# DmitryUlyanov/deep-image-prior

Measured on NVIDIA H100. Metric: optimisation iterations/sec (512x512 skip-net denoising, sum over independent images), higher is better.
Workload: dtype fp32 storage; tf32 tensor-core multiplies with fp32 accumulate in the convs (cuDNN's default fp32 mode)

## Files before the change

deep-image-prior_b200/csrc/conv_tc.cu:

```cuda
#include "conv_tc.cuh"
#include "ptx.cuh"
#include "wgmma.cuh"
#include "kernels.cuh"

namespace dip {

static constexpr int kTileM = 128;
static constexpr int kABytes = kTileM * 128;
static constexpr int kChunkBytes = kTileM * 128;
static constexpr int kNumThreads = 256;
static constexpr int kAccStride = kAccS;

struct SmemCtl {
  uint64_t full[8];
  uint64_t empty[8];
  float bias[160];
};

__host__ __device__ constexpr int round32(int n) { return (n + 31) & ~31; }
__host__ __device__ constexpr int round1024(int n) { return (n + 1023) & ~1023; }

template <bool BF16, int NT>
__device__ __forceinline__ void tc_conv_consumer(const TcConvParams& p, const TcConvParams* pm, SmemCtl* ctl,
                                                 uint8_t* stage_base, int stage_bytes, uint8_t* staging, int n_iters,
                                                 int tile0, int tile_stride, int num_tiles, int tiles_pp, int n_off) {
  const int et = threadIdx.x - 128;
  const int w = et >> 5, lane = et & 31;
  float acc[2][NT / 2];
  int stage = 0;
  uint32_t phase = 0;
  double stat_s1 = 0.0, stat_s2 = 0.0;
  const int bw_shift = 31 - __clz(p.bw);
  const uint32_t base_lo = desc_lo(smem_u32(stage_base));
  const uint32_t stage_step = static_cast<uint32_t>(stage_bytes) >> 4;
  constexpr uint32_t kBOff = static_cast<uint32_t>(kABytes) >> 4;
  constexpr uint32_t kHalfOff = (64u * 128u) >> 4;
  for (int it = 0; it < n_iters; ++it) {
    const int tile = tile0 + it * tile_stride;
    int tx = tile % p.tiles_x, ty = tile / p.tiles_x;
    int opx = 0, opy = 0;
    int kb_per_tile = p.kh * p.kw * p.kblocks;
    if (p.nphase > 0) {
      if (tile >= num_tiles) break;
      const int t = tile % tiles_pp;
      tx = t % p.tiles_x; ty = t / p.tiles_x;
      const TcConvParams::Phase& q = p.phs[tile / tiles_pp];
      opx = q.opx; opy = q.opy;
      kb_per_tile = q.kh * q.kw * p.kblocks;
    }
    const int x0 = tx * p.bw, y0 = ty * p.bh;
#pragma unroll
    for (int i = 0; i < NT / 2; ++i) { acc[0][i] = 0.f; acc[1][i] = 0.f; }
    int prev = -1;
    for (int kbt = 0; kbt < kb_per_tile; ++kbt) {
      mbar_wait(&ctl->full[stage], phase);
      const uint32_t a_lo = base_lo + stage * stage_step;
      const uint32_t b_lo = a_lo + kBOff;
      wgmma_fence();
#pragma unroll
      for (int k = 0; k < 4; ++k) {
        wgmma_ss<NT, BF16>(acc[0], desc_of(a_lo + 2 * k), desc_of(b_lo + 2 * k));
        wgmma_ss<NT, BF16>(acc[1], desc_of(a_lo + kHalfOff + 2 * k), desc_of(b_lo + 2 * k));
      }
      wgmma_commit();
      if (prev >= 0) {
        wgmma_wait<1>();
        if (lane == 0) mbar_arrive(&ctl->empty[prev]);
      }
      prev = stage;
      if (++stage == p.stages) { stage = 0; phase ^= 1; }
    }
    wgmma_wait<0>();
    if (prev >= 0 && lane == 0) mbar_arrive(&ctl->empty[prev]);

    if (et == 0) tma_store_wait_read0();
    named_bar_sync(1, 128);
#pragma unroll
    for (int h = 0; h < 2; ++h) {
#pragma unroll
      for (int j = 0; j < NT / 8; ++j) {
        const int col = 8 * j + 2 * (lane & 3);
        const int chunk = col >> 5;
        if (chunk < p.n_chunks) {
          const int q = (col & 31) >> 2, e = col & 3;
#pragma unroll
          for (int rr = 0; rr < 2; ++rr) {
            const int row = 64 * h + 16 * w + (lane >> 2) + 8 * rr;
            float2 o;
            o.x = acc[h][4 * j + 2 * rr] + ctl->bias[col];
            o.y = acc[h][4 * j + 2 * rr + 1] + ctl->bias[col + 1];
            *reinterpret_cast<float2*>(staging + chunk * kChunkBytes + row * 128 + ((q ^ (row & 7)) << 4) + e * 4) = o;
          }
        }
      }
    }
    fence_proxy_async_smem();
    named_bar_sync(1, 128);
    if (et == 0) {
      if (p.nphase > 0)
        for (int j = 0; j < p.n_chunks; ++j) tma_store_5d(&pm->tmD, staging + j * kChunkBytes, n_off + j * 32, opx, x0, opy, y0);
      else
        for (int j = 0; j < p.n_chunks; ++j) tma_store_3d(&pm->tmD, staging + j * kChunkBytes, n_off + j * 32, x0, y0);
      tma_store_commit();
    }
    if (p.stats != nullptr && et < p.n_mma) {
      const int c = et;
      const int j = c >> 5, q = (c & 31) >> 2, e = c & 3;
      const uint8_t* cb = staging + j * kChunkBytes + e * 4;
      float a0 = 0.f, a1 = 0.f, b0 = 0.f, b1 = 0.f;
      if (x0 + p.bw <= p.out_w && y0 + p.bh <= p.out_h) {
#pragma unroll 8
        for (int m = 0; m < kTileM; m += 2) {
          const float x = *reinterpret_cast<const float*>(cb + m * 128 + ((q ^ (m & 7)) << 4));
          const float y = *reinterpret_cast<const float*>(cb + (m + 1) * 128 + ((q ^ ((m + 1) & 7)) << 4));
          a0 += x; b0 = fmaf(x, x, b0);
          a1 += y; b1 = fmaf(y, y, b1);
        }
      } else {
        for (int m = 0; m < kTileM; ++m) {
          const int py = m >> bw_shift, px = m & (p.bw - 1);
          if (x0 + px < p.out_w && y0 + py < p.out_h) {
            const float x = *reinterpret_cast<const float*>(cb + m * 128 + ((q ^ (m & 7)) << 4));
            a0 += x; b0 = fmaf(x, x, b0);
          }
        }
      }
      stat_s1 += static_cast<double>(a0 + a1);
      stat_s2 += static_cast<double>(b0 + b1);
    }
  }
  if (p.stats != nullptr && et < p.n_mma && n_off + et < p.stats_ld) {
    const int rep = (blockIdx.x % kAccR) * kAccLine;
    atomicAdd(&p.stats[(n_off + et) * kAccStride + rep], stat_s1);
    atomicAdd(&p.stats[(p.stats_ld + n_off + et) * kAccStride + rep], stat_s2);
  }
  if (et == 0) tma_store_wait_all0();
}

template <bool DEEP, bool BF16 = false>
__device__ __forceinline__ void tc_conv_body(const TcConvParams& p, const TcConvParams* pm, uint8_t* smem_raw) {
  constexpr int KE = BF16 ? 64 : 32;
  const int grid_x = DEEP ? p.vgrid : static_cast<int>(gridDim.x);
  if (DEEP && static_cast<int>(blockIdx.x) >= grid_x) return;
  uint8_t* smem = reinterpret_cast<uint8_t*>((reinterpret_cast<uintptr_t>(smem_raw) + 1023) & ~uintptr_t(1023));
  const int nt = round32(p.n_mma);
  const int b_bytes = p.n_mma * 128;
  const int stage_bytes = kABytes + round1024(nt * 128);
  uint8_t* stage_base = smem;
  uint8_t* staging = stage_base + p.stages * stage_bytes;
  SmemCtl* ctl = reinterpret_cast<SmemCtl*>(staging + p.n_chunks * kChunkBytes);

  const int warp = threadIdx.x >> 5;
  const int lane = threadIdx.x & 31;
  const int tiles_pp = p.tiles_x * p.tiles_y;
  const int num_tiles = p.nphase > 0 ? tiles_pp * p.nphase : tiles_pp;
  const int n_split = p.n_split < 1 ? 1 : p.n_split;
  const int n_part = blockIdx.x % n_split;
  const int n_off = n_part * p.n_mma;
  const int n_total = p.n_mma * n_split;
  const int tile_stride = grid_x / n_split;
  const int n_iters = (num_tiles + tile_stride - 1) / tile_stride;
  const int tile0 = blockIdx.x / n_split;

  if (!DEEP) pdl_trigger();
  if (warp == 0 && lane == 0) {
    tma_prefetch_desc(&pm->tmA);
    tma_prefetch_desc(&pm->tmB);
    tma_prefetch_desc(&pm->tmD);
  }
  if (warp == 1 && lane == 0) {
    for (int i = 0; i < p.stages; ++i) {
      mbar_init(&ctl->full[i], 1);
      mbar_init(&ctl->empty[i], 4);
    }
    fence_mbar_init();
  }
  if (!DEEP) pdl_wait();
  if (warp == 3) {
    for (int i = lane; i < 160; i += 32)
      ctl->bias[i] = (p.bias != nullptr && i < p.n_mma && (p.n_valid == 0 || n_off + i < p.n_valid)) ? p.bias[n_off + i] : 0.f;
  }
  __syncthreads();

  if (warp == 0) {
    int stage = 0;
    uint32_t phase = 0;
    for (int it = 0; it < n_iters; ++it) {
      const int tile = tile0 + it * tile_stride;
      int kh = p.kh, kw = p.kw, offx = p.offx, offy = p.offy, tap0 = 0;
      int x0 = (tile % p.tiles_x) * p.bw, y0 = (tile / p.tiles_x) * p.bh;
      if (p.nphase > 0) {
        if (tile >= num_tiles) break;
        const TcConvParams::Phase& q = p.phs[tile / tiles_pp];
        const int t = tile % tiles_pp;
        kh = q.kh; kw = q.kw; offx = q.offx; offy = q.offy; tap0 = q.tap0;
        x0 = (t % p.tiles_x) * p.bw; y0 = (t / p.tiles_x) * p.bh;
      }
      for (int r = 0; r < kh; ++r) {
        for (int s = 0; s < kw; ++s) {
          const int ix = offx + s, iy = offy + r;
          int cpx, cx, cpy, cy;
          if (p.stride == 1) {
            cpx = 0; cx = x0 + ix; cpy = 0; cy = y0 + iy;
          } else {
            cpx = ix & 1; cx = x0 + (ix >> 1); cpy = iy & 1; cy = y0 + (iy >> 1);
          }
          const int tap = tap0 + r * kw + s;
          for (int kb = 0; kb < p.kblocks; ++kb) {
            mbar_wait(&ctl->empty[stage], phase ^ 1);
            uint8_t* sa = stage_base + stage * stage_bytes;
            if (elect_one()) {
              mbar_expect_tx(&ctl->full[stage], kABytes + b_bytes);
              tma_load_5d(sa, &pm->tmA, &ctl->full[stage], kb * KE, cpx, cx, cpy, cy);
              tma_load_2d(sa + kABytes, &pm->tmB, &ctl->full[stage], kb * KE, tap * n_total + n_off);
            }
            __syncwarp();
            if (++stage == p.stages) { stage = 0; phase ^= 1; }
          }
        }
      }
    }
  } else if (warp >= 4) {
    switch (nt) {
      case 32: tc_conv_consumer<BF16, 32>(p, pm, ctl, stage_base, stage_bytes, staging, n_iters, tile0, tile_stride, num_tiles, tiles_pp, n_off); break;
      case 64: tc_conv_consumer<BF16, 64>(p, pm, ctl, stage_base, stage_bytes, staging, n_iters, tile0, tile_stride, num_tiles, tiles_pp, n_off); break;
      case 96: tc_conv_consumer<BF16, 96>(p, pm, ctl, stage_base, stage_bytes, staging, n_iters, tile0, tile_stride, num_tiles, tiles_pp, n_off); break;
      case 128: tc_conv_consumer<BF16, 128>(p, pm, ctl, stage_base, stage_bytes, staging, n_iters, tile0, tile_stride, num_tiles, tiles_pp, n_off); break;
      default: tc_conv_consumer<BF16, 160>(p, pm, ctl, stage_base, stage_bytes, staging, n_iters, tile0, tile_stride, num_tiles, tiles_pp, n_off); break;
    }
  }
  __syncthreads();
}
__global__ void __launch_bounds__(kNumThreads, 1) tc_conv_kernel(const __grid_constant__ TcConvParams p) {
  extern __shared__ __align__(1024) uint8_t smem_raw[];
  tc_conv_body<false>(p, &p, smem_raw);
}
__global__ void __launch_bounds__(kNumThreads, 1) tc_conv_kernel_bf16(const __grid_constant__ TcConvParams p) {
  extern __shared__ __align__(1024) uint8_t smem_raw[];
  tc_conv_body<false, true>(p, &p, smem_raw);
}

struct SmemCtlW {
  uint64_t full[8];
  uint64_t empty[8];
  uint64_t bt_full[2];
  uint64_t bt_empty[2];
};

__host__ __device__ constexpr int wgrad_tbuf_bytes(bool bf16, int n_cols) {
  return (bf16 ? kTileM * 128 : 0) + round1024(n_cols * 128);
}


template <int NT>
__device__ __forceinline__ void tc_wgrad_transposer(const TcWgradParams& p, SmemCtlW* ctl, uint32_t stage_base, int stage_bytes,
                                                    uint32_t bt_base, int items) {
  constexpr int kBt = wgrad_tbuf_bytes(false, NT);
  constexpr int kUnitsO = ((NT + 31) / 32) * 8;
  constexpr int kIters = (kUnitsO + 11) / 12;
  constexpr int y_bytes = 4 * kWgradKp * 128;
  const int tt = threadIdx.x - 32;
  const int lane = threadIdx.x & 31;
  const int b = tt & 7, b0 = b & 1, b1 = (b >> 1) & 1, b2 = b >> 2;
  uint32_t src[kIters], dst[kIters], sq[kIters], dq[kIters];
  bool ok[kIters];
#pragma unroll
  for (int it = 0; it < kIters; ++it) {
    const int o = (tt >> 3) + 12 * it;
    const int kk = (b1 ^ (o & 1)) | ((b2 ^ ((o >> 1) & 1)) << 1);
    const int c4 = (o >> 3) * 8 + b2 * 4 + b1 * 2 + ((o >> 2) & 1);
    ok[it] = o < kUnitsO && c4 < NT / 4;
    src[it] = y_bytes + (c4 >> 3) * (kWgradKp * 128) + (8 * kk + b0) * 128;
    sq[it] = (c4 & 7) ^ b0;
    dst[it] = c4 * 4 * 128;
    dq[it] = (2 * kk + b0) ^ ((c4 & 1) << 2);
  }
  int stage = 0, tb = 0;
  uint32_t phase = 0, tphase = 0;
  for (int item = blockIdx.x; item < items; item += gridDim.x) {
    const int ks = item % p.ksplits;
    const int blk0 = static_cast<int>((static_cast<long long>(p.px_blocks) * ks) / p.ksplits);
    const int blk1 = static_cast<int>((static_cast<long long>(p.px_blocks) * (ks + 1)) / p.ksplits);
    for (int blk = blk0; blk < blk1; ++blk) {
      mbar_wait(&ctl->full[stage], phase);
      mbar_wait(&ctl->bt_empty[tb], tphase ^ 1);
      const uint32_t sx = stage_base + stage * stage_bytes;
      const uint32_t bt = bt_base + tb * kBt;
#pragma unroll
      for (int it = 0; it < kIters; ++it) {
        if (ok[it]) {
          uint4 v[4];
#pragma unroll
          for (int i = 0; i < 4; ++i) v[i] = lds128(sx + src[it] + 256 * i + ((sq[it] ^ (2 * i)) << 4));
          sts128(bt + dst[it] + ((dq[it] ^ 0) << 4), v[0].x, v[1].x, v[2].x, v[3].x);
          sts128(bt + dst[it] + 128 + ((dq[it] ^ 1) << 4), v[0].y, v[1].y, v[2].y, v[3].y);
          sts128(bt + dst[it] + 256 + ((dq[it] ^ 2) << 4), v[0].z, v[1].z, v[2].z, v[3].z);
          sts128(bt + dst[it] + 384 + ((dq[it] ^ 3) << 4), v[0].w, v[1].w, v[2].w, v[3].w);
        }
      }
      fence_proxy_async_smem();
      mbar_arrive(&ctl->bt_full[tb]);
      __syncwarp();
      if (lane == 0) mbar_arrive(&ctl->empty[stage]);
      if (++stage == p.stages) { stage = 0; phase ^= 1; }
      tb ^= 1;
      if (tb == 0) tphase ^= 1;
    }
  }
}

template <int NT, bool DOUBLE>
__device__ __forceinline__ void tc_wgrad_mma(const TcWgradParams& p, SmemCtlW* ctl, uint32_t stage_base, int stage_bytes,
                                             uint32_t bt_base, int items) {
  constexpr int kBt = wgrad_tbuf_bytes(false, NT);
  constexpr bool kDouble = DOUBLE && NT <= 136;
  const int et = threadIdx.x - 128;
  const int w = et >> 5, lane = et & 31, g = lane >> 2, t = lane & 3;
  const int taps = p.kh * p.kw;
  uint32_t aoff[4];
#pragma unroll
  for (int r = 0; r < 4; ++r) {
    const int hi = r & 1, e = r >> 1;
    const int q = 4 * (w & 1) + (g >> 2) + 2 * hi, px = 2 * t + e;
    aoff[r] = (w >> 1) * (kWgradKp * 128) + px * 128 + ((q ^ px) << 4) + (g & 3) * 4;
  }
  auto load_a = [&](uint32_t (&f)[8][4], uint32_t sy) {
#pragma unroll
    for (int h = 0; h < 2; ++h)
#pragma unroll
      for (int kk = 0; kk < 4; ++kk)
#pragma unroll
        for (int r = 0; r < 4; ++r) f[4 * h + kk][r] = lds32(sy + aoff[r] + h * 2 * (kWgradKp * 128) + kk * 1024);
  };
  int stage = 0, tb = 0;
  uint32_t phase = 0, tphase = 0;
  bool pending = false;
  float acc[2][NT / 2];
  uint32_t fa[8][4], fb[8][4];
  auto step = [&](uint32_t (&cur)[8][4], uint32_t (&nxt)[8][4], bool more) {
    mbar_wait(&ctl->bt_full[tb], tphase);
    const uint32_t b_lo = desc_lo(bt_base + tb * kBt);
    wgmma_fence();
#pragma unroll
    for (int kk = 0; kk < 4; ++kk) {
      wgmma_rs<NT>(acc[0], cur[kk], desc_of(b_lo + 2 * kk));
      wgmma_rs<NT>(acc[1], cur[4 + kk], desc_of(b_lo + 2 * kk));
    }
    wgmma_commit();
    __syncwarp();
    if (lane == 0) mbar_arrive(&ctl->empty[stage]);
    if (++stage == p.stages) { stage = 0; phase ^= 1; }
    if constexpr (kDouble) wgmma_wait<1>(); else wgmma_wait<0>();
    if (pending && lane == 0) mbar_arrive(&ctl->bt_empty[tb ^ 1]);
    pending = true;
    tb ^= 1;
    if (tb == 0) tphase ^= 1;
    if (more) {
      mbar_wait(&ctl->full[stage], phase);
      load_a(nxt, stage_base + stage * stage_bytes);
    }
  };
  for (int item = blockIdx.x; item < items; item += gridDim.x) {
    const int tap = item / p.ksplits, ks = item % p.ksplits;
    const int blk0 = static_cast<int>((static_cast<long long>(p.px_blocks) * ks) / p.ksplits);
    const int blk1 = static_cast<int>((static_cast<long long>(p.px_blocks) * (ks + 1)) / p.ksplits);
#pragma unroll
    for (int i = 0; i < NT / 2; ++i) { acc[0][i] = 0.f; acc[1][i] = 0.f; }
    if (blk0 < blk1) {
      mbar_wait(&ctl->full[stage], phase);
      load_a(fa, stage_base + stage * stage_bytes);
    }
    for (int blk = blk0; blk < blk1; blk += 2) {
      step(fa, kDouble ? fb : fa, blk + 1 < blk1);
      if (blk + 1 == blk1) break;
      step(kDouble ? fb : fa, fa, blk + 2 < blk1);
    }
    wgmma_wait<0>();
    if (pending && lane == 0) mbar_arrive(&ctl->bt_empty[tb ^ 1]);
    pending = false;
    float* dst = p.partial + (static_cast<size_t>(ks) * taps + tap) * 128 * NT;
#pragma unroll
    for (int h = 0; h < 2; ++h) {
#pragma unroll
      for (int j = 0; j < NT / 8; ++j) {
        const int col = 8 * j + 2 * t;
#pragma unroll
        for (int rr = 0; rr < 2; ++rr) {
          const int n = 64 * h + 16 * w + g + 8 * rr;
          *reinterpret_cast<float2*>(dst + static_cast<size_t>(n) * NT + col) =
              make_float2(acc[h][4 * j + 2 * rr], acc[h][4 * j + 2 * rr + 1]);
        }
      }
    }
  }
}

template <int NT>
__device__ __forceinline__ void tc_wgrad_consumer_bf16(const TcWgradParams& p, SmemCtlW* ctl, uint8_t* smem, int stage_bytes,
                                                       uint8_t* tbase, int items) {
  constexpr int KE = 64;
  constexpr int E = 2;
  constexpr int kTA = kTileM * 128;
  constexpr int kTBuf = wgrad_tbuf_bytes(true, NT);
  constexpr int kRows = 128 + NT;
  const int et = threadIdx.x - 128;
  const int w = et >> 5, lane = et & 31;
  constexpr int chunk_bytes = kWgradKp * 128;
  constexpr int y_bytes = (128 / KE) * chunk_bytes;
  constexpr int groups = kWgradKp * E / 16;
  constexpr int nk = kWgradKp / 16;
  const int taps = p.kh * p.kw;
  int stage = 0, tb = 0;
  uint32_t phase = 0;
  float acc[2][NT / 2];
  for (int item = blockIdx.x; item < items; item += gridDim.x) {
    const int tap = item / p.ksplits, ks = item % p.ksplits;
    const int blk0 = static_cast<int>((static_cast<long long>(p.px_blocks) * ks) / p.ksplits);
    const int blk1 = static_cast<int>((static_cast<long long>(p.px_blocks) * (ks + 1)) / p.ksplits);
#pragma unroll
    for (int i = 0; i < NT / 2; ++i) { acc[0][i] = 0.f; acc[1][i] = 0.f; }
    for (int blk = blk0; blk < blk1; ++blk) {
      mbar_wait(&ctl->full[stage], phase);
      named_bar_sync(1, 128);
      const uint8_t* sy = smem + stage * stage_bytes;
      const uint8_t* sx = sy + y_bytes;
      uint8_t* ta = tbase + tb * kTBuf;
      uint8_t* tbb = ta + kTA;
      for (int i = et; i < kRows * groups; i += 128) {
        const int g = i / kRows, row = i % kRows;
        const bool is_y = row < 128;
        const int rs = is_y ? row : row - 128;
        const uint8_t* src = (is_y ? sy : sx) + (rs / KE) * chunk_bytes;
        const int cb = (rs % KE) * E;
        uint32_t v[4];
#pragma unroll
        for (int u = 0; u < 4; ++u) {
          const int px = g * 8 + 2 * u;
          const uint32_t lo = *reinterpret_cast<const uint16_t*>(src + px * 128 + ((((cb >> 4) ^ (px & 7)) << 4) | (cb & 15)));
          const uint32_t hi = *reinterpret_cast<const uint16_t*>(src + (px + 1) * 128 + ((((cb >> 4) ^ ((px + 1) & 7)) << 4) | (cb & 15)));
          v[u] = lo | (hi << 16);
        }
        uint8_t* dst = (is_y ? ta : tbb) + rs * 128 + ((g ^ (rs & 7)) << 4);
        *reinterpret_cast<uint4*>(dst) = make_uint4(v[0], v[1], v[2], v[3]);
      }
      fence_proxy_async_smem();
      named_bar_sync(1, 128);
      if (lane == 0) mbar_arrive(&ctl->empty[stage]);
      const uint32_t a_lo = desc_lo(smem_u32(ta)), b_lo = desc_lo(smem_u32(tbb));
      wgmma_fence();
#pragma unroll
      for (int k = 0; k < nk; ++k) {
        wgmma_ss<NT, true>(acc[0], desc_of(a_lo + 2 * k), desc_of(b_lo + 2 * k));
        wgmma_ss<NT, true>(acc[1], desc_of(a_lo + ((64u * 128u) >> 4) + 2 * k), desc_of(b_lo + 2 * k));
      }
      wgmma_commit();
      wgmma_wait<1>();
      tb ^= 1;
      if (++stage == p.stages) { stage = 0; phase ^= 1; }
    }
    wgmma_wait<0>();
    float* dst = p.partial + (static_cast<size_t>(ks) * taps + tap) * 128 * NT;
#pragma unroll
    for (int h = 0; h < 2; ++h) {
#pragma unroll
      for (int j = 0; j < NT / 8; ++j) {
        const int col = 8 * j + 2 * (lane & 3);
#pragma unroll
        for (int rr = 0; rr < 2; ++rr) {
          const int n = 64 * h + 16 * w + (lane >> 2) + 8 * rr;
          *reinterpret_cast<float2*>(dst + static_cast<size_t>(n) * NT + col) =
              make_float2(acc[h][4 * j + 2 * rr], acc[h][4 * j + 2 * rr + 1]);
        }
      }
    }
  }
}

template <bool DEEP, bool BF16, int NT>
__device__ __forceinline__ void tc_wgrad_role(const TcWgradParams& p, SmemCtlW* ctl, uint8_t* smem, int stage_bytes,
                                              uint8_t* tbase, int items, int warp) {
  if constexpr (BF16) {
    if (warp >= 4) tc_wgrad_consumer_bf16<NT>(p, ctl, smem, stage_bytes, tbase, items);
  } else {
    if (warp >= 4) tc_wgrad_mma<NT, !DEEP>(p, ctl, smem_u32(smem), stage_bytes, smem_u32(tbase), items);
    else tc_wgrad_transposer<NT>(p, ctl, smem_u32(smem), stage_bytes, smem_u32(tbase), items);
  }
}

template <bool DEEP, bool BF16 = false>
__device__ __forceinline__ void tc_wgrad_body(const TcWgradParams& p, const TcWgradParams* pm, uint8_t* smem_raw) {
  uint8_t* smem = reinterpret_cast<uint8_t*>((reinterpret_cast<uintptr_t>(smem_raw) + 1023) & ~uintptr_t(1023));
  constexpr int KE = BF16 ? 64 : 32;
  constexpr int YCH = 128 / KE;
  constexpr int chunk_bytes = kWgradKp * 128;
  const int y_bytes = YCH * chunk_bytes;
  const int x_bytes = p.c_chunks * chunk_bytes;
  const int stage_bytes = y_bytes + x_bytes;
  uint8_t* tbase = smem + p.stages * stage_bytes;
  SmemCtlW* ctl = reinterpret_cast<SmemCtlW*>(tbase + 2 * wgrad_tbuf_bytes(BF16, p.n_cols));
  const int items = p.kh * p.kw * p.ksplits;

  const int warp = threadIdx.x >> 5;
  const int lane = threadIdx.x & 31;
  if (!DEEP) pdl_trigger();
  if (warp == 0 && lane == 0) {
    tma_prefetch_desc(&pm->tmY);
    tma_prefetch_desc(&pm->tmX);
  }
  if (warp == 1 && lane == 0) {
    for (int i = 0; i < p.stages; ++i) {
      mbar_init(&ctl->full[i], 1);
      mbar_init(&ctl->empty[i], BF16 ? 4 : 7);
    }
    for (int i = 0; i < 2; ++i) {
      mbar_init(&ctl->bt_full[i], 96);
      mbar_init(&ctl->bt_empty[i], 4);
    }
    fence_mbar_init();
  }
  if (!DEEP) pdl_wait();
  __syncthreads();

  if (warp == 0) {
    int stage = 0;
    uint32_t phase = 0;
    for (int item = blockIdx.x; item < items; item += gridDim.x) {
      const int tap = item / p.ksplits, ks = item % p.ksplits;
      const int r = tap / p.kw, s = tap % p.kw;
      const int blk0 = static_cast<int>((static_cast<long long>(p.px_blocks) * ks) / p.ksplits);
      const int blk1 = static_cast<int>((static_cast<long long>(p.px_blocks) * (ks + 1)) / p.ksplits);
      const int ix = p.offx + s, iy = p.offy + r;
      for (int blk = blk0; blk < blk1; ++blk) {
        const int y = blk / p.px_blocks_x;
        const int x0 = (blk % p.px_blocks_x) * kWgradKp;
        int cpx, cx, cpy, cy;
        if (p.stride == 1) {
          cpx = 0; cx = x0 + ix; cpy = 0; cy = y + iy;
        } else {
          cpx = ix & 1; cx = x0 + (ix >> 1); cpy = iy & 1; cy = y + (iy >> 1);
        }
        mbar_wait(&ctl->empty[stage], phase ^ 1);
        uint8_t* sy = smem + stage * stage_bytes;
        if (elect_one()) {
          mbar_expect_tx(&ctl->full[stage], stage_bytes);
          for (int j = 0; j < YCH; ++j) tma_load_3d(sy + j * chunk_bytes, &pm->tmY, &ctl->full[stage], j * KE, x0, y);
          for (int j = 0; j < p.c_chunks; ++j)
            tma_load_5d(sy + y_bytes + j * chunk_bytes, &pm->tmX, &ctl->full[stage], j * KE, cpx, cx, cpy, cy);
        }
        __syncwarp();
        if (++stage == p.stages) { stage = 0; phase ^= 1; }
      }
    }
  } else {
    switch (p.n_cols) {
      case 32: tc_wgrad_role<DEEP, BF16, 32>(p, ctl, smem, stage_bytes, tbase, items, warp); break;
      case 64: tc_wgrad_role<DEEP, BF16, 64>(p, ctl, smem, stage_bytes, tbase, items, warp); break;
      case 96: tc_wgrad_role<DEEP, BF16, 96>(p, ctl, smem, stage_bytes, tbase, items, warp); break;
      case 128: tc_wgrad_role<DEEP, BF16, 128>(p, ctl, smem, stage_bytes, tbase, items, warp); break;
      case 136: tc_wgrad_role<DEEP, BF16, 136>(p, ctl, smem, stage_bytes, tbase, items, warp); break;
      default: tc_wgrad_role<DEEP, BF16, 160>(p, ctl, smem, stage_bytes, tbase, items, warp); break;
    }
  }
  __syncthreads();
}
__global__ void __launch_bounds__(kNumThreads, 1) tc_wgrad_kernel(const __grid_constant__ TcWgradParams p) {
  extern __shared__ __align__(1024) uint8_t smem_raw[];
  tc_wgrad_body<false>(p, &p, smem_raw);
}
__global__ void __launch_bounds__(kNumThreads, 1) tc_wgrad_kernel_bf16(const __grid_constant__ TcWgradParams p) {
  extern __shared__ __align__(1024) uint8_t smem_raw[];
  tc_wgrad_body<false, true>(p, &p, smem_raw);
}

static constexpr size_t kMaxSmem = 232448;

size_t tc_conv_smem_bytes(const TcConvParams& p) {
  const size_t b_bytes = round1024(round32(p.n_mma) * 128);
  return 1024 + p.stages * (kABytes + b_bytes) + static_cast<size_t>(p.n_chunks) * kChunkBytes + sizeof(SmemCtl);
}
size_t tc_wgrad_smem_bytes(const TcWgradParams& p) {
  const size_t chunk = static_cast<size_t>(kWgradKp) * 128;
  const size_t tbuf = wgrad_tbuf_bytes(p.bf16 != 0, p.n_cols);
  return 1024 + p.stages * ((p.bf16 ? 2 : 4) * chunk + static_cast<size_t>(p.c_chunks) * chunk) + 2 * tbuf + sizeof(SmemCtlW);
}

cudaError_t tc_kernels_init() {
  cudaError_t e = cudaFuncSetAttribute(tc_conv_kernel, cudaFuncAttributeMaxDynamicSharedMemorySize, (int)kMaxSmem);
  if (e != cudaSuccess) return e;
  e = cudaFuncSetAttribute(tc_conv_kernel_bf16, cudaFuncAttributeMaxDynamicSharedMemorySize, (int)kMaxSmem);
  if (e != cudaSuccess) return e;
  e = cudaFuncSetAttribute(tc_wgrad_kernel_bf16, cudaFuncAttributeMaxDynamicSharedMemorySize, (int)kMaxSmem);
  if (e != cudaSuccess) return e;
  return cudaFuncSetAttribute(tc_wgrad_kernel, cudaFuncAttributeMaxDynamicSharedMemorySize, (int)kMaxSmem);
}

static bool conv_params_ok(const TcConvParams& p) {
  return p.n_mma >= 1 && p.n_mma <= 160 && p.n_chunks == (p.n_mma + 31) / 32 && p.stages >= 1 && p.stages <= 8 &&
         p.kblocks >= 1 && p.nphase >= 0 && p.nphase <= 4 &&
         (p.bw & (p.bw - 1)) == 0 && p.bw * p.bh == kTileM;
}

cudaError_t tc_conv_launch(const TcConvParams& p, int num_sms, cudaStream_t s) {
  if (!conv_params_ok(p)) return cudaErrorInvalidValue;
  const int tiles = p.tiles_x * p.tiles_y * (p.nphase > 0 ? p.nphase : 1);
  int grid = tiles < num_sms ? tiles : num_sms;
  if (p.n_split > 1) {
    if (tiles * p.n_split > num_sms) return cudaErrorInvalidValue;
    grid = tiles * p.n_split;
  }
  const size_t smem = tc_conv_smem_bytes(p);
  if (smem > kMaxSmem) return cudaErrorInvalidValue;
  return launch_k(p.bf16 ? tc_conv_kernel_bf16 : tc_conv_kernel, dim3(grid), dim3(kNumThreads), smem, s, 1, p);
}
int tc_conv_grid(const TcConvParams& p, int num_sms) {
  const int tiles = p.tiles_x * p.tiles_y * (p.nphase > 0 ? p.nphase : 1);
  if (p.n_split > 1) return tiles * p.n_split;
  return tiles < num_sms ? tiles : num_sms;
}

cudaError_t tc_wgrad_launch(const TcWgradParams& p, cudaStream_t s) {
  const size_t smem = tc_wgrad_smem_bytes(p);
  const bool cols_ok = p.n_cols == 32 || p.n_cols == 64 || p.n_cols == 96 || p.n_cols == 128 || p.n_cols == 136 ||
                       p.n_cols == 160;
  if (smem > kMaxSmem || !cols_ok || p.n_cols > p.c_chunks * (p.bf16 ? 64 : 32) || p.stages < 1 || p.stages > 8)
    return cudaErrorInvalidValue;
  return launch_k(p.bf16 ? tc_wgrad_kernel_bf16 : tc_wgrad_kernel, dim3(p.kh * p.kw * p.ksplits), dim3(kNumThreads), smem, s, 1, p);
}

}
```

deep-image-prior_b200/csrc/conv_tc.cuh:

```cuda
#pragma once
#include <cuda.h>
#include <cuda_runtime.h>
#include <stdint.h>

namespace dip {

struct TcConvParams {
  CUtensorMap tmA;
  CUtensorMap tmB;
  CUtensorMap tmD;
  int tiles_x, tiles_y;
  int bw, bh;
  int out_w, out_h;
  int kh, kw;
  int stride;
  int offx, offy;
  int bf16;
  int kblocks;
  int n_mma;
  int n_chunks;
  int stages;
  int n_split;
  int vgrid;
  int nphase;
  struct Phase { int kh, kw, offx, offy, tap0, opx, opy; } phs[4];
  int n_valid;
  const float* bias;
  double* stats;
  int stats_ld;
};

static constexpr int kWgradKp = 32;
struct TcWgradParams {
  CUtensorMap tmY;
  CUtensorMap tmX;
  float* partial;
  int kh, kw, stride, offx, offy;
  int px_blocks_x;
  int px_blocks;
  int bf16;
  int c_chunks;
  int n_cols;
  int ksplits;
  int stages;
};

size_t tc_conv_smem_bytes(const TcConvParams& p);
size_t tc_wgrad_smem_bytes(const TcWgradParams& p);
cudaError_t tc_conv_launch(const TcConvParams& p, int num_sms, cudaStream_t s);
cudaError_t tc_wgrad_launch(const TcWgradParams& p, cudaStream_t s);
int tc_conv_grid(const TcConvParams& p, int num_sms);
cudaError_t tc_kernels_init();

}
```

deep-image-prior_b200/csrc/engine.cu:

```cuda
#include <cuda.h>
#include <cuda_bf16.h>
#include <cuda_runtime.h>
#include <math.h>
#include <stdio.h>
#include <stdlib.h>
#include <string.h>

#include <initializer_list>
#include <map>
#include <string>
#include <vector>

#include "../../include/dip.h"
#include "conv_tc.cuh"
#include "deep.cuh"
#include "kernels.cuh"

namespace dip {

static thread_local std::string g_err;
static int fail(const std::string& m) {
  g_err = m;
  return -1;
}
#define DIP_CUDA(expr)                                                                                   \
  do {                                                                                                   \
    cudaError_t _e = (expr);                                                                             \
    if (_e != cudaSuccess) return fail(std::string(#expr) + ": " + cudaGetErrorString(_e));              \
  } while (0)
#define DIP_CHECK(expr)        \
  do {                         \
    int _r = (expr);           \
    if (_r != 0) return _r;    \
  } while (0)

typedef CUresult (*PFN_encodeTiled)(CUtensorMap*, CUtensorMapDataType, cuuint32_t, void*, const cuuint64_t*,
                                    const cuuint64_t*, const cuuint32_t*, const cuuint32_t*, CUtensorMapInterleave,
                                    CUtensorMapSwizzle, CUtensorMapL2promotion, CUtensorMapFloatOOBfill);
static PFN_encodeTiled g_encode = nullptr;
static int g_num_sms = 0;
static unsigned long long g_inited_mask = 0;

static int engine_init() {
  int dev = 0;
  DIP_CUDA(cudaGetDevice(&dev));
  if (dev >= 64) return fail("dip: device ordinal >= 64 not supported");
  if (g_inited_mask & (1ull << dev)) return 0;
  cudaDeviceProp prop;
  DIP_CUDA(cudaGetDeviceProperties(&prop, dev));
  if (prop.major != 9 || prop.minor != 0)
    return fail("dip requires an sm_90 (H100) device; found sm_" + std::to_string(prop.major * 10 + prop.minor));
  g_num_sms = prop.multiProcessorCount;
  void* fn = nullptr;
  cudaDriverEntryPointQueryResult q;
  DIP_CUDA(cudaGetDriverEntryPoint("cuTensorMapEncodeTiled", &fn, cudaEnableDefault, &q));
  if (fn == nullptr || q != cudaDriverEntryPointSuccess) return fail("cuTensorMapEncodeTiled not available from the driver");
  g_encode = reinterpret_cast<PFN_encodeTiled>(fn);
  DIP_CUDA(tc_kernels_init());
  DIP_CUDA(down_kernels_init());
  DIP_CUDA(deep_kernels_init());
  g_inited_mask |= 1ull << dev;
  return 0;
}

static bool is_tc(int prec) { return prec == DIP_PRECISION_TF32 || prec == DIP_PRECISION_BF16; }

static int encode_map(CUtensorMap* m, const void* base, int rank, const cuuint64_t* dims, const cuuint64_t* strides_b,
                      const cuuint32_t* box, bool bf16 = false) {
  cuuint32_t estr[5] = {1, 1, 1, 1, 1};
  CUresult r = g_encode(m, bf16 ? CU_TENSOR_MAP_DATA_TYPE_BFLOAT16 : CU_TENSOR_MAP_DATA_TYPE_FLOAT32, rank, const_cast<void*>(base), dims, strides_b, box, estr,
                        CU_TENSOR_MAP_INTERLEAVE_NONE, CU_TENSOR_MAP_SWIZZLE_128B,
                        CU_TENSOR_MAP_L2_PROMOTION_L2_128B,
                        CU_TENSOR_MAP_FLOAT_OOB_FILL_NONE);
  if (r != CUDA_SUCCESS) {
    char buf[256];
    snprintf(buf, sizeof buf, "cuTensorMapEncodeTiled failed (%d): rank %d dims %llu %llu %llu box %u %u %u", (int)r, rank,
             (unsigned long long)dims[0], (unsigned long long)dims[1], (unsigned long long)(rank > 2 ? dims[2] : 0), box[0],
             box[1], rank > 2 ? box[2] : 0);
    return fail(buf);
  }
  return 0;
}
static int map_act5(CUtensorMap* m, const void* base, int rows, int cols, int ld, int c, int stride, int bw, int bh,
                    bool bf16 = false) {
  const cuuint64_t e = bf16 ? 2 : sizeof(float);
  cuuint64_t dims[5], str[4];
  if (stride == 1) {
    dims[0] = c; dims[1] = 1; dims[2] = cols; dims[3] = 1; dims[4] = rows;
    str[0] = ld * e; str[1] = ld * e; str[2] = (cuuint64_t)cols * ld * e; str[3] = (cuuint64_t)cols * ld * e;
  } else {
    dims[0] = c; dims[1] = 2; dims[2] = cols / 2; dims[3] = 2; dims[4] = rows / 2;
    str[0] = ld * e; str[1] = 2 * ld * e; str[2] = (cuuint64_t)cols * ld * e; str[3] = 2 * (cuuint64_t)cols * ld * e;
  }
  cuuint32_t box[5] = {bf16 ? 64u : 32u, 1, (cuuint32_t)bw, 1, (cuuint32_t)bh};
  return encode_map(m, base, 5, dims, str, box, bf16);
}
static int map_act3(CUtensorMap* m, const void* base, int rows, int cols, int ld, int c, int bw, int bh, bool bf16 = false) {
  const cuuint64_t e = bf16 ? 2 : sizeof(float);
  cuuint64_t dims[3] = {(cuuint64_t)c, (cuuint64_t)cols, (cuuint64_t)rows};
  cuuint64_t str[2] = {ld * e, (cuuint64_t)cols * ld * e};
  cuuint32_t box[3] = {bf16 ? 64u : 32u, (cuuint32_t)bw, (cuuint32_t)bh};
  return encode_map(m, base, 3, dims, str, box, bf16);
}
static int map_w2(CUtensorMap* m, const void* base, int rows_total, int kcols, int box_rows, bool bf16 = false) {
  const cuuint64_t e = bf16 ? 2 : sizeof(float);
  cuuint64_t dims[2] = {(cuuint64_t)kcols, (cuuint64_t)rows_total};
  cuuint64_t str[1] = {kcols * e};
  cuuint32_t box[2] = {bf16 ? 64u : 32u, (cuuint32_t)box_rows};
  return encode_map(m, base, 2, dims, str, box, bf16);
}

static void pick_tile(int w, int h, int* bw, int* bh) {
  const int cand[5][2] = {{128, 1}, {64, 2}, {32, 4}, {16, 8}, {8, 16}};
  long long best = -1;
  for (int i = 0; i < 5; ++i) {
    const long long cw = (w + cand[i][0] - 1) / cand[i][0] * cand[i][0];
    const long long ch = (h + cand[i][1] - 1) / cand[i][1] * cand[i][1];
    const long long cost = cw * ch * 64 + (cand[i][0] + cand[i][1]);
    if (best < 0 || cost < best) { best = cost; *bw = cand[i][0]; *bh = cand[i][1]; }
  }
}
static int round_up(int x, int m) { return (x + m - 1) / m * m; }
struct Timer {
  bool on = false;
  std::vector<cudaEvent_t> pool;
  size_t used = 0;
  struct Rec { int cls; double flops; size_t e0, e1; };
  std::vector<Rec> recs;
  size_t get(cudaStream_t s) {
    if (used == pool.size()) { cudaEvent_t e; cudaEventCreate(&e); pool.push_back(e); }
    cudaEventRecord(pool[used], s);
    return used++;
  }
  void reset() { used = 0; recs.clear(); }
};
struct TimeScope {
  Timer* t; int cls; double flops; size_t e0 = 0; cudaStream_t s;
  TimeScope(Timer* t_, int cls_, double flops_, cudaStream_t s_) : t(t_ && t_->on ? t_ : nullptr), cls(cls_), flops(flops_), s(s_) {
    if (t) e0 = t->get(s);
  }
  ~TimeScope() { if (t) { size_t e1 = t->get(s); t->recs.push_back({cls, flops, e0, e1}); } }
};

enum HbmId { H_INPUT_PAD = 0, H_NOISE, H_SKINNY_FWD, H_BN_ACT_WRITE, H_BN_ACT_HEAD, H_CAT_STATS, H_CAT_WRITE, H_BN_BWD_REDUCE,
             H_BN_BWD_APPLY, H_CAT_BWD_REDUCE, H_CAT_BWD_APPLY, H_UPADJ, H_SKINNY_BWD, H_MSE, H_ADAM, H_HEAD_DLOGIT, H_DOWN_FWD,
             H_DOWN_BWD, H_PACK, H_WGRAD_REDUCE };
#define HBM_T(timer, id, sub, bytes, s, stmt)                                              \
  do {                                                                                     \
    TimeScope _ts((timer), 16 + 8 * (int)(id) + (int)(sub), (double)(bytes), (s));         \
    stmt;                                                                                  \
  } while (0)

static int pick_nsplit(int tiles, int n_rows) {
  int mx = 4;
  if (const char* e = getenv("DIP_NSPLIT_MAX")) mx = atoi(e);
  int sp = 1;
  while (sp * 2 <= mx && tiles * sp * 2 <= g_num_sms && n_rows % (32 * sp * 2) == 0) sp *= 2;
  return sp;
}
static void fit_stages(TcConvParams& p, size_t budget = 232448) {
  p.stages = 6;
  while (tc_conv_smem_bytes(p) > budget && p.stages > 2) p.stages--;
}
struct ConvOp {
  Timer* timer = nullptr;
  double alg_flops() const { return 2.0 * out_h * out_w * (double)N * C * k * k; }
  int N = 128, C = 0, k = 1, stride = 1, rot = 0;
  int Np = 128;
  int n_pad = 128;
  int n_pad16 = 128;
  int Ctot = 0, coff = 0;
  bool do_fprop = true, do_wgrad = true;
  int dg_ld = 0;
  int c_pad = 0;
  int crows = 0;
  bool bf16 = false;
  int c_pad16 = 0;
  const uint16_t* in16 = nullptr; int in_ld16 = 0;
  const uint16_t* dg_in16 = nullptr;
  const uint16_t* wg_dy16 = nullptr;
  const float* in = nullptr; int in_rows = 0, in_cols = 0, in_ld = 0; int offx = 0, offy = 0;
  float* out = nullptr; int out_h = 0, out_w = 0;
  double* stats = nullptr;
  float* wp_f = nullptr; float* wp_d = nullptr;
  float* wacc = nullptr;
  bool has_dgrad = false;
  bool dg_s2 = false;
  const float* dg_in = nullptr; int dg_in_h = 0, dg_in_w = 0;
  float* dg_out = nullptr; int dg_out_h = 0, dg_out_w = 0; int dg_off = 0;
  const float* wg_dy = nullptr; int wg_h = 0, wg_w = 0;
  int p_w = -1, p_b = -1;
  TcConvParams fp{}, dg{};
  TcWgradParams wg{};
  int simt_ksplits = 1;

  void set_shapes() {
    c_pad = round_up(C, 32);
    c_pad16 = round_up(C, 64);
    crows = round_up(C, 16);
    Np = round_up(N, 16); n_pad = round_up(N, 32); n_pad16 = round_up(N, 64);
    if (Ctot == 0) Ctot = C;
    if (dg_ld == 0) dg_ld = C;
  }
  size_t wp_f_elems() const { return (size_t)k * k * Np * c_pad; }
  size_t wp_d_elems() const { return (size_t)k * k * crows * n_pad; }
  size_t wacc_elems() const { return (size_t)tc_ksplits() * k * k * 128 * wg_cols(); }
  int wg_cols() const { return C > 128 && C <= 136 ? 136 : c_pad; }
  int tc_ksplits() const {
    const int blocks = wg_h * ((wg_w + kWgradKp - 1) / kWgradKp);
    int ks = static_cast<int>(kNumSms) / (k * k);
    if (ks > blocks) ks = blocks;
    return ks < 1 ? 1 : ks;
  }
  size_t partial_elems(int prec) const {
    return is_tc(prec) ? wacc_elems() : (size_t)simt_ksplits * k * k * 128 * c_pad;
  }

  int build_tc(float* partial) {
    int bw, bh;
    pick_tile(out_w, out_h, &bw, &bh);
    fp = TcConvParams{};
    if (do_fprop) {
    DIP_CHECK(bf16 ? map_act5(&fp.tmA, in16, in_rows, in_cols, in_ld16, C, stride, bw, bh, true)
                   : map_act5(&fp.tmA, in, in_rows, in_cols, in_ld, C, stride, bw, bh));
    fp.n_split = pick_nsplit(((out_w + bw - 1) / bw) * ((out_h + bh - 1) / bh), Np);
    DIP_CHECK(map_w2(&fp.tmB, wp_f, k * k * Np, bf16 ? c_pad16 : c_pad, Np / fp.n_split, bf16));
    DIP_CHECK(map_act3(&fp.tmD, out, out_h, out_w, N, N, bw, bh));
    fp.tiles_x = (out_w + bw - 1) / bw; fp.tiles_y = (out_h + bh - 1) / bh;
    fp.bw = bw; fp.bh = bh; fp.out_w = out_w; fp.out_h = out_h;
    fp.kh = fp.kw = k; fp.stride = stride; fp.offx = offx; fp.offy = offy;
    fp.bf16 = bf16 ? 1 : 0;
    fp.kblocks = bf16 ? c_pad16 / 64 : c_pad / 32;
    fp.n_mma = Np / fp.n_split; fp.n_chunks = (fp.n_mma + 31) / 32;
    fp.n_valid = N;
    fp.bias = nullptr; fp.stats = stats; fp.stats_ld = N;
    fit_stages(fp);
    }
    if (has_dgrad && dg_s2) {
      const int gh = dg_out_h / 2, gw = dg_out_w / 2;
      pick_tile(gw, gh, &bw, &bh);
      dg = TcConvParams{};
      DIP_CHECK(bf16 ? map_act5(&dg.tmA, dg_in16, dg_in_h, dg_in_w, N, N, 1, bw, bh, true)
                     : map_act5(&dg.tmA, dg_in, dg_in_h, dg_in_w, N, N, 1, bw, bh));
      dg.n_split = pick_nsplit(4 * ((gw + bw - 1) / bw) * ((gh + bh - 1) / bh), crows);
      DIP_CHECK(map_w2(&dg.tmB, wp_d, k * k * crows, bf16 ? n_pad16 : n_pad, crows / dg.n_split, bf16));
      DIP_CHECK(map_act5(&dg.tmD, dg_out, dg_out_h, dg_out_w, dg_ld, C, 2, bw, bh));
      dg.tiles_x = (gw + bw - 1) / bw; dg.tiles_y = (gh + bh - 1) / bh;
      dg.bw = bw; dg.bh = bh; dg.out_w = gw; dg.out_h = gh;
      dg.kh = dg.kw = 2; dg.stride = 1; dg.offx = dg.offy = -1;
      dg.nphase = 4;
      int t0 = 0;
      for (int a = 0; a < 2; ++a)
        for (int b = 0; b < 2; ++b) {
          TcConvParams::Phase& q = dg.phs[a * 2 + b];
          q.kh = 2 - a; q.kw = 2 - b; q.offy = a == 0 ? -1 : 0; q.offx = b == 0 ? -1 : 0; q.tap0 = t0; q.opx = b; q.opy = a;
          t0 += q.kh * q.kw;
        }
      dg.bf16 = bf16 ? 1 : 0;
      dg.kblocks = bf16 ? n_pad16 / 64 : n_pad / 32;
      dg.n_mma = crows / dg.n_split; dg.n_chunks = (dg.n_mma + 31) / 32;
      dg.bias = nullptr; dg.stats = nullptr; dg.stats_ld = 0;
      fit_stages(dg);
    } else if (has_dgrad) {
      pick_tile(dg_out_w, dg_out_h, &bw, &bh);
      dg = TcConvParams{};
      DIP_CHECK(bf16 ? map_act5(&dg.tmA, dg_in16, dg_in_h, dg_in_w, N, N, 1, bw, bh, true)
                     : map_act5(&dg.tmA, dg_in, dg_in_h, dg_in_w, N, N, 1, bw, bh));
      dg.n_split = pick_nsplit(((dg_out_w + bw - 1) / bw) * ((dg_out_h + bh - 1) / bh), crows);
      DIP_CHECK(map_w2(&dg.tmB, wp_d, k * k * crows, bf16 ? n_pad16 : n_pad, crows / dg.n_split, bf16));
      DIP_CHECK(map_act3(&dg.tmD, dg_out, dg_out_h, dg_out_w, dg_ld, C, bw, bh));
      dg.tiles_x = (dg_out_w + bw - 1) / bw; dg.tiles_y = (dg_out_h + bh - 1) / bh;
      dg.bw = bw; dg.bh = bh; dg.out_w = dg_out_w; dg.out_h = dg_out_h;
      dg.kh = dg.kw = k; dg.stride = 1; dg.offx = dg.offy = dg_off;
      dg.bf16 = bf16 ? 1 : 0;
      dg.kblocks = bf16 ? n_pad16 / 64 : n_pad / 32;
      dg.n_mma = crows / dg.n_split; dg.n_chunks = (dg.n_mma + 31) / 32;
      dg.bias = nullptr; dg.stats = nullptr; dg.stats_ld = 0;
      fit_stages(dg);
    }
    wg = TcWgradParams{};
    if (!do_wgrad) return 0;
    wg.bf16 = bf16 ? 1 : 0;
    if (bf16) {
      DIP_CHECK(map_act3(&wg.tmY, wg_dy16, wg_h, wg_w, N, N, kWgradKp, 1, true));
      DIP_CHECK(map_act5(&wg.tmX, in16, in_rows, in_cols, in_ld16, C, stride, kWgradKp, 1, true));
    } else {
      DIP_CHECK(map_act3(&wg.tmY, wg_dy, wg_h, wg_w, N, N, kWgradKp, 1));
      DIP_CHECK(map_act5(&wg.tmX, in, in_rows, in_cols, in_ld, C, stride, kWgradKp, 1));
    }
    wg.partial = partial;
    wg.kh = wg.kw = k; wg.stride = stride; wg.offx = offx; wg.offy = offy;
    wg.px_blocks_x = (wg_w + kWgradKp - 1) / kWgradKp;
    wg.px_blocks = wg_h * wg.px_blocks_x;
    wg.c_chunks = bf16 ? c_pad16 / 64 : c_pad / 32;
    wg.n_cols = wg_cols();
    wg.ksplits = tc_ksplits();
    wg.stages = 6;
    while (tc_wgrad_smem_bytes(wg) > 232448 && wg.stages > 1) wg.stages--;
    if (tc_wgrad_smem_bytes(wg) > 232448) return fail("wgrad stage does not fit in shared memory");
    return 0;
  }

  int run_fprop(int prec, const float* bias, cudaStream_t s) {
    if (is_tc(prec)) {
      TcConvParams p = fp;
      p.bias = bias;
      TimeScope ts(timer, 0, alg_flops(), s);
      DIP_CUDA(tc_conv_launch(p, g_num_sms, s));
    } else {
      SimtConvArgs a{};
      a.A = in; a.a_h = in_rows; a.a_w = in_cols; a.a_ld = in_ld; a.a_c = C;
      a.Wp = wp_f; a.n_rows = Np; a.c_pad = c_pad;
      a.D = out; a.d_h = out_h; a.d_w = out_w; a.d_ld = N; a.d_c = N;
      a.kh = a.kw = k; a.stride = stride; a.offx = offx; a.offy = offy; a.bias = bias;
      launch_simt_conv(a, s);
      if (stats != nullptr) launch_channel_stats(out, N, N, out_h * out_w, stats, s);
      DIP_CUDA(cudaGetLastError());
    }
    return 0;
  }
  int run_dgrad(int prec, cudaStream_t s) {
    if (is_tc(prec)) {
      TimeScope ts(timer, 1, alg_flops(), s);
      DIP_CUDA(tc_conv_launch(dg, g_num_sms, s));
    } else {
      SimtConvArgs a{};
      a.A = dg_in; a.a_h = dg_in_h; a.a_w = dg_in_w; a.a_ld = N; a.a_c = N;
      a.Wp = wp_d; a.n_rows = crows; a.c_pad = n_pad;
      a.D = dg_out; a.d_h = dg_out_h; a.d_w = dg_out_w; a.d_ld = dg_ld; a.d_c = C;
      a.kh = a.kw = k; a.stride = 1; a.offx = a.offy = dg_off; a.bias = nullptr;
      launch_simt_conv(a, s);
      DIP_CUDA(cudaGetLastError());
    }
    return 0;
  }
  int run_wgrad(int prec, float* partial, float* dw, cudaStream_t s) {
    static const bool dbg_skip = getenv("DIP_DBG_SKIP_WGRAD") != nullptr;
    if (dbg_skip) return 0;
    int ks;
    if (is_tc(prec)) {
      TcWgradParams p = wg;
      p.partial = wacc != nullptr ? wacc : partial;
      {
        TimeScope ts(timer, 2, alg_flops(), s);
        DIP_CUDA(tc_wgrad_launch(p, s));
      }
      if (wacc != nullptr) return 0;
      launch_wgrad_reduce(partial, p.ksplits, N, C, k, k, rot, p.n_cols, dw, s, Ctot, coff);
      DIP_CUDA(cudaGetLastError());
      return 0;
    } else {
      SimtWgradArgs a{};
      a.dY = wg_dy; a.h = wg_h; a.w = wg_w; a.dy_ld = N; a.n = N;
      a.X = in; a.x_h = in_rows; a.x_w = in_cols; a.x_ld = in_ld; a.x_c = C;
      a.kh = a.kw = k; a.stride = stride; a.offx = offx; a.offy = offy;
      a.partial = partial; a.c_pad = c_pad; a.ksplits = ks = simt_ksplits;
      launch_simt_wgrad(a, s);
    }
    HBM_T(timer, H_WGRAD_REDUCE, 0, ((double)ks + 1.0) * k * k * 128.0 * c_pad * sizeof(float), s,
          launch_wgrad_reduce(partial, ks, N, C, k, k, rot, c_pad, dw, s, Ctot, coff));
    DIP_CUDA(cudaGetLastError());
    return 0;
  }
};

struct PackEntry {
  const float* w; float* dst_f; float* dst_d;
  int N, C, k, rot, n_rows, c_pad, c_rows;
  int Ctot, coff;
  int s2;
  int bf16;
  int c_pad16;
  int n_pad;
};
__constant__ int kS2Taps[9] = {2 * 3 + 2, 2 * 3 + 0, 0 * 3 + 2, 0 * 3 + 0,
                               2 * 3 + 1, 0 * 3 + 1,
                               1 * 3 + 2, 1 * 3 + 0,
                               1 * 3 + 1};
__global__ void k_pack_table(const PackEntry* __restrict__ tab) {
  pdl_enter();
  const PackEntry e = tab[blockIdx.y];
  const int taps = e.k * e.k;
  const int c_pad = e.bf16 ? e.c_pad16 : e.c_pad;
  __nv_bfloat16* const f16 = reinterpret_cast<__nv_bfloat16*>(e.dst_f);
  __nv_bfloat16* const d16 = reinterpret_cast<__nv_bfloat16*>(e.dst_d);
  const long long nf = e.dst_f != nullptr ? (long long)taps * e.n_rows * c_pad : 0;
  const int n_pad = e.n_pad > 0 ? e.n_pad : 128;
  const long long nd = e.dst_d != nullptr ? (long long)taps * e.c_rows * n_pad : 0;
  for (long long i = (long long)blockIdx.x * blockDim.x + threadIdx.x; i < nf + nd; i += (long long)gridDim.x * blockDim.x) {
    if (i < nf) {
      const int c = (int)(i % c_pad), n = (int)((i / c_pad) % e.n_rows), tap = (int)(i / ((long long)c_pad * e.n_rows));
      float v = 0.f;
      if (n < e.N && c < e.C) v = e.w[((long long)n * e.Ctot + (c + e.coff + e.rot) % e.Ctot) * taps + tap];
      if (e.bf16) f16[i] = __float2bfloat16_rn(v); else e.dst_f[i] = v;
    } else {
      const long long j = i - nf;
      const int n = (int)(j % n_pad), c = (int)((j / n_pad) % e.c_rows), tapf = (int)(j / ((long long)n_pad * e.c_rows));
      const int tap = e.s2 ? kS2Taps[tapf] : taps - 1 - tapf;
      float v = 0.f;
      if (n < e.N && c < e.C) v = e.w[((long long)n * e.Ctot + (c + e.coff + e.rot) % e.Ctot) * taps + tap];
      if (e.bf16) d16[j] = __float2bfloat16_rn(v); else e.dst_d[j] = v;
    }
  }
}
struct UnpackEntry {
  const float* acc; float* dw;
  int N, C, taps, rot, cols, Ctot, coff, ks;
};
__global__ void k_wgrad_unpack_table(const UnpackEntry* __restrict__ tab) {
  pdl_enter();
  const UnpackEntry e = tab[blockIdx.y];
  const int total = e.N * e.C * e.taps;
  for (int i = blockIdx.x * blockDim.x + threadIdx.x; i < total; i += gridDim.x * blockDim.x) {
    const int tap = i % e.taps, c = (i / e.taps) % e.C, n = i / (e.taps * e.C);
    const size_t split = (size_t)e.taps * 128 * e.cols;
    const float* src = e.acc + ((size_t)tap * 128 + n) * e.cols + c;
    float v = 0.f;
    for (int k = 0; k < e.ks; ++k) v += src[k * split];
    e.dw[((size_t)n * e.Ctot + (c + e.coff + e.rot) % e.Ctot) * e.taps + tap] = v;
  }
}
struct CvtEntry {
  const double* src; float* dst; int n, rot;
  int row, row_ld;
};
__global__ void k_cvt_table(const CvtEntry* __restrict__ tab) {
  pdl_enter();
  const CvtEntry e = tab[blockIdx.x];
  for (int i = threadIdx.x; i < e.n; i += blockDim.x) {
    const int si = e.row > 0 ? (i / e.row) * e.row_ld + i % e.row : i;
    e.dst[(i + e.rot) % e.n] = (float)acc_get(e.src + (size_t)si * kAccS);
  }
}
struct RunEntry {
  const double* fwd; float* rm; float* rv; void* nb; int C, rot; float n; int nb_is_float;
};
__global__ void k_running_table(const RunEntry* __restrict__ tab) {
  pdl_enter();
  const RunEntry e = tab[blockIdx.x];
  if (e.rm == nullptr) return;
  for (int c = threadIdx.x; c < e.C; c += blockDim.x) {
    const int ct = (c + e.rot) % e.C;
    const double m = acc_get(e.fwd + c * kAccS) / e.n;
    double var = acc_get(e.fwd + (e.C + c) * kAccS) / e.n - m * m;
    if (var < 0) var = 0;
    const double unb = e.n > 1.f ? var * e.n / (e.n - 1.0) : var;
    e.rm[ct] = 0.9f * e.rm[ct] + 0.1f * (float)m;
    e.rv[ct] = 0.9f * e.rv[ct] + 0.1f * (float)unb;
  }
  if (threadIdx.x == 0 && e.nb != nullptr) {
    if (e.nb_is_float) *reinterpret_cast<float*>(e.nb) += 1.f; else *reinterpret_cast<long long*>(e.nb) += 1;
  }
}

struct Arena {
  uint8_t* base;
  size_t off = 0;
  template <typename T>
  T* get(size_t n) {
    off = (off + 255) & ~size_t(255);
    T* p = base ? reinterpret_cast<T*>(base + off) : nullptr;
    off += n * sizeof(T);
    return p;
  }
};
struct BufInfo {
  void* ptr; int rows, cols, ld, c;
};
struct BnLayer {
  int C = 0, rot = 0; float n = 1.f;
  double* fwd = nullptr; double* bwd = nullptr; double* dbias = nullptr;
  int p_gamma = -1, p_beta = -1, p_bias = -1, idx = -1;
};
struct Level {
  int H, W, h, w, Cin;
  int Cin_act;
  int bilinear;
  int nd = 128, nu = 128, ns = 0, cu = 128;
  float *rawF = nullptr, *dRawF = nullptr;
  uint16_t* dRawF16 = nullptr;
  float *Pin, *raw_s, *raw_d1, *P_d1, *raw_d2, *P_d2, *P_cat, *raw_u, *A_u, *raw_v, *U;
  uint16_t *Pin16 = nullptr, *P_d1_16 = nullptr, *P_d2_16 = nullptr, *P_cat16 = nullptr, *A_u16 = nullptr;
  uint16_t *dRaw_v16 = nullptr, *dRaw_u16 = nullptr, *dRaw_d2_16 = nullptr, *dRaw_d1_16 = nullptr, *dRaw_s16 = nullptr;
  int Pin_ld16 = 0, cat_ld16 = 0;
  float *dUp;
  float *dS;
  float *dRaw_v, *dA_u, *dRaw_u, *dP_cat, *dCat, *dRaw_s, *dRaw_d2, *dP_d1, *dRaw_d1, *ZS, *dPin;
  BnLayer bn_s, bn_d1, bn_d2, bn_cat, bn_u, bn_v;
  int p_skip_w, p_skip_b;
  double* dw_s;
  ConvOp d1, d2, up, c11;
  ConvOp sk, up_a, up_b;
};

}

using namespace dip;

struct dip_plan {
  dip_net_desc desc;
  int H, W;
  int zero_pad = 0;
  bool dry = false;
  uint8_t* ws = nullptr;
  size_t ws_bytes = 0;
  std::vector<Level> lv;
  std::vector<long long> numel;
  std::vector<float*> params, grads;
  std::vector<void*> running;
  std::vector<BnLayer*> bns;
  std::vector<ConvOp*> convs;
  std::map<std::string, BufInfo> bufs;
  int p_head_w = -1, p_head_b = -1;
  double* dw_head = nullptr; double* db_head = nullptr; double* db_scratch = nullptr;
  float* out_saved = nullptr;
  double* acc_fwd = nullptr; size_t acc_fwd_n = 0;
  double* acc_bwd = nullptr; size_t acc_bwd_n = 0;
  float* partial = nullptr;
  float* zbuf = nullptr; float* dout = nullptr; float* dl4 = nullptr;
  static constexpr int kDownMaxK = 64;
  float* ds_kern = nullptr;
  float* ds_y = nullptr;
  float* ds_dy = nullptr;
  int ds_K = 0, ds_f = 1, ds_pad = 0, ds_Ho = 0, ds_Wo = 0;
  static constexpr int kLossRing = 65536;
  double* loss_ring = nullptr;
  int* it_dev = nullptr;
  struct GraphKey {
    const void *z0 = nullptr, *target = nullptr, *mask = nullptr, *out = nullptr, *slots = nullptr;
    unsigned long long adam_id = 0, adam_bind = 0;
    float sigma = 0.f; uint64_t seed = 0; double lr = 0.0;
    bool operator==(const GraphKey& o) const {
      return z0 == o.z0 && target == o.target && mask == o.mask && out == o.out && slots == o.slots && adam_id == o.adam_id &&
             adam_bind == o.adam_bind && sigma == o.sigma && seed == o.seed && lr == o.lr;
    }
  };
  GraphKey gkey{};
  cudaGraphExec_t gexec = nullptr;
  cudaGraphExec_t gfwd = nullptr, gbwd = nullptr;
  cudaStream_t gstream = nullptr;
  cudaEvent_t gev_in = nullptr, gev_out = nullptr;
  cudaStream_t wstream = nullptr;
  cudaStream_t sstream = nullptr;
  std::vector<cudaEvent_t> wev;
  size_t wev_used = 0;
  bool side_on = false;
  std::vector<dip::ConvOp*> deferred;
  struct { bool on = false; const float* z0 = nullptr; float sigma = 0.f; uint64_t seed = 0, offset = 0; const int* it_dev = nullptr; } fnoise;
  bool prepacked = false;
  PackEntry* d_pack = nullptr; CvtEntry* d_cvt = nullptr; RunEntry* d_run = nullptr; UnpackEntry* d_unpack = nullptr;
  int n_pack = 0, n_cvt = 0, n_run = 0, n_unpack = 0;
  float* wacc_base = nullptr; size_t wacc_bytes = 0;
  static constexpr int kDeepMaxOps = 96;
  DeepOp* d_deep_fwd = nullptr; DeepOp* d_deep_bwd = nullptr;
  int n_deep_fwd = 0, n_deep_bwd = 0, deep_grid = 0, deep_from = 2;
  unsigned* deep_bar = nullptr;
  long long pack_max = 0;
  bool bound = false;
  int nbt_is_float = 0;
  int launches_fwd = 0, launches_bwd = 0;
  Timer timer;
};

namespace dip {

static BnRef bn_ref(const dip_plan* P, const BnLayer& b) {
  BnRef r;
  r.fwd = b.fwd; r.gamma = P->params[b.p_gamma]; r.beta = P->params[b.p_beta];
  r.C = b.C; r.rot = b.rot; r.inv_n = 1.f / b.n;
  return r;
}

static int build_plan(dip_plan* P, Arena& A) {
  const dip_net_desc& d = P->desc;
  const int L = d.num_scales;
  if (L < 1 || L > 8) return fail("dip-b200: 1..8 scales supported");
  std::vector<int> ND(L), NU(L), NS(L);
  for (int l = 0; l < L; ++l) {
    ND[l] = d.channels > 0 ? d.channels : d.channels_down[l];
    NU[l] = d.channels > 0 ? d.channels : d.channels_up[l];
    NS[l] = d.channels > 0 ? d.skip_channels : d.channels_skip[l];
    for (int w : {ND[l], NU[l]})
      if (w < 8 || w > 128 || w % 8 != 0)
        return fail("dip-b200: num_channels_down / num_channels_up must be multiples of 8 in [8, 128] (128 in the BASELINE configurations)");
  }
  bool wide = true, uniform = true;
  for (int l = 0; l < L; ++l) {
    wide = wide && NS[l] == 128 && ND[l] == 128 && NU[l] == 128;
    uniform = uniform && ND[l] == 128 && NU[l] == 128 && NS[l] == NS[0];
  }
  for (int l = 0; l < L; ++l)
    if (!(wide || NS[l] == 0 || NS[l] == 4))
      return fail("dip-b200: num_channels_skip must be 0 or 4 per scale, or 128 at every scale of a 128-wide network");
  const int CS = NS[0];
  if (d.downsample_mode != 0 && d.downsample_mode != 1) return fail("dip-b200: downsample_mode must be 'stride' (0) or 'avg' (1)");
  const bool avg = d.downsample_mode == 1;
  auto psl = [&](int l) { return NS[l] > 0 ? 4 : 0; };
  if (d.in_channels < 1 || d.in_channels > 128) return fail("dip-b200: input depth must be in [1,128]");
  int cin_eng = 4;
  while (cin_eng < d.in_channels) cin_eng *= 2;
  if (d.out_channels < 1 || d.out_channels > 4) return fail("dip-b200: num_output_channels must be <= 4");
  if (P->H % (1 << L) || P->W % (1 << L)) return fail("dip-b200: H and W must be divisible by 2^num_scales");
  if ((P->H >> L) < 2 || (P->W >> L) < 2)
    return fail("dip-b200: H and W must be at least 2 * 2^num_scales (ReflectionPad2d(1) in front of the deepest 3x3 conv needs 2 "
                "pixels per side: torch raises for the reference's network as well)");
  const int prec = d.precision;
  if (prec != DIP_PRECISION_TF32 && prec != DIP_PRECISION_FP32 && prec != DIP_PRECISION_BF16) return fail("dip-b200: unknown precision");
  const bool bf = prec == DIP_PRECISION_BF16;
  P->lv.resize(L);
  int pidx = 0;
  std::vector<int> pre(L), post(L);
  {
    int idx = 0;
    for (int l = 0; l < L; ++l) { pre[l] = idx; idx += 8 + psl(l); }
    for (int l = L - 1; l >= 0; --l) { post[l] = idx; idx += 10; }
    P->p_head_w = idx; P->p_head_b = idx + 1;
    pidx = idx + 2;
  }
  P->numel.assign(pidx, 0);
  P->bns.clear(); P->convs.clear();
  size_t acc_f = 0, acc_b = 0;
  auto bn_init = [&](BnLayer& b, int C, int rot, int n, int pg, int pbias) {
    b.C = C; b.rot = rot; b.n = (float)n; b.p_gamma = pg; b.p_beta = pg + 1; b.p_bias = pbias;
    P->numel[pg] = C; P->numel[pg + 1] = C;
    acc_f += 2 * C; acc_b += 3 * C;
  };
  for (int l = 0; l < L; ++l) {
// ... 1347 lines not shown
```

deep-image-prior_b200/csrc/ptx.cuh:

```cuda
#pragma once
#include <cuda_runtime.h>
#include <cuda.h>
#include <stdint.h>

namespace dip {

__device__ __forceinline__ uint32_t smem_u32(const void* p) {
  return static_cast<uint32_t>(__cvta_generic_to_shared(p));
}

__device__ __forceinline__ uint32_t lds32(uint32_t addr) {
  uint32_t v;
  asm volatile("ld.shared.b32 %0, [%1];" : "=r"(v) : "r"(addr) : "memory");
  return v;
}
__device__ __forceinline__ uint4 lds128(uint32_t addr) {
  uint4 v;
  asm volatile("ld.shared.v4.b32 {%0, %1, %2, %3}, [%4];" : "=r"(v.x), "=r"(v.y), "=r"(v.z), "=r"(v.w) : "r"(addr) : "memory");
  return v;
}
__device__ __forceinline__ void sts128(uint32_t addr, uint32_t a, uint32_t b, uint32_t c, uint32_t d) {
  asm volatile("st.shared.v4.b32 [%0], {%1, %2, %3, %4};" ::"r"(addr), "r"(a), "r"(b), "r"(c), "r"(d) : "memory");
}

__device__ __forceinline__ uint32_t elect_one() {
  uint32_t pred = 0;
  asm volatile(
      "{\n\t.reg .b32 rx;\n\t.reg .pred px;\n\t"
      "elect.sync rx|px, 0xffffffff;\n\t"
      "selp.b32 %0, 1, 0, px;\n\t}\n"
      : "=r"(pred));
  return pred;
}

__device__ __forceinline__ void mbar_init(uint64_t* bar, uint32_t count) {
  asm volatile("mbarrier.init.shared::cta.b64 [%0], %1;" ::"r"(smem_u32(bar)), "r"(count));
}
__device__ __forceinline__ void fence_mbar_init() {
  asm volatile("fence.mbarrier_init.release.cluster;" ::: "memory");
}
__device__ __forceinline__ void mbar_expect_tx(uint64_t* bar, uint32_t bytes) {
  asm volatile("mbarrier.arrive.expect_tx.shared::cta.b64 _, [%0], %1;" ::"r"(smem_u32(bar)), "r"(bytes)
               : "memory");
}
__device__ __forceinline__ void mbar_arrive(uint64_t* bar) {
  asm volatile("mbarrier.arrive.shared::cta.b64 _, [%0];" ::"r"(smem_u32(bar)) : "memory");
}
__device__ __forceinline__ void mbar_wait(uint64_t* bar, uint32_t parity) {
  asm volatile(
      "{\n\t.reg .pred p;\n\t"
      "WAIT_LOOP:\n\t"
      "mbarrier.try_wait.parity.shared::cta.b64 p, [%0], %1;\n\t"
      "@p bra WAIT_DONE;\n\t"
      "bra WAIT_LOOP;\n\t"
      "WAIT_DONE:\n\t}\n" ::"r"(smem_u32(bar)),
      "r"(parity)
      : "memory");
}

__device__ __forceinline__ void fence_proxy_async_smem() {
  asm volatile("fence.proxy.async.shared::cta;" ::: "memory");
}

__device__ __forceinline__ void tma_prefetch_desc(const CUtensorMap* m) {
  asm volatile("prefetch.tensormap [%0];" ::"l"(reinterpret_cast<uint64_t>(m)) : "memory");
}
__device__ __forceinline__ void tma_load_2d(void* dst, const CUtensorMap* m, uint64_t* bar, int c0, int c1) {
  asm volatile(
      "cp.async.bulk.tensor.2d.shared::cluster.global.tile.mbarrier::complete_tx::bytes "
      "[%0], [%1, {%3, %4}], [%2];" ::"r"(smem_u32(dst)),
      "l"(reinterpret_cast<uint64_t>(m)), "r"(smem_u32(bar)), "r"(c0), "r"(c1)
      : "memory");
}
__device__ __forceinline__ void tma_load_3d(void* dst, const CUtensorMap* m, uint64_t* bar, int c0, int c1,
                                            int c2) {
  asm volatile(
      "cp.async.bulk.tensor.3d.shared::cluster.global.tile.mbarrier::complete_tx::bytes "
      "[%0], [%1, {%3, %4, %5}], [%2];" ::"r"(smem_u32(dst)),
      "l"(reinterpret_cast<uint64_t>(m)), "r"(smem_u32(bar)), "r"(c0), "r"(c1), "r"(c2)
      : "memory");
}
__device__ __forceinline__ void tma_load_5d(void* dst, const CUtensorMap* m, uint64_t* bar, int c0, int c1,
                                            int c2, int c3, int c4) {
  asm volatile(
      "cp.async.bulk.tensor.5d.shared::cluster.global.tile.mbarrier::complete_tx::bytes "
      "[%0], [%1, {%3, %4, %5, %6, %7}], [%2];" ::"r"(smem_u32(dst)),
      "l"(reinterpret_cast<uint64_t>(m)), "r"(smem_u32(bar)), "r"(c0), "r"(c1), "r"(c2), "r"(c3), "r"(c4)
      : "memory");
}
__device__ __forceinline__ void tma_store_3d(const CUtensorMap* m, const void* src, int c0, int c1, int c2) {
  asm volatile(
      "cp.async.bulk.tensor.3d.global.shared::cta.tile.bulk_group [%0, {%2, %3, %4}], [%1];" ::"l"(
          reinterpret_cast<uint64_t>(m)),
      "r"(smem_u32(src)), "r"(c0), "r"(c1), "r"(c2)
      : "memory");
}
__device__ __forceinline__ void tma_store_5d(const CUtensorMap* m, const void* src, int c0, int c1, int c2, int c3, int c4) {
  asm volatile(
      "cp.async.bulk.tensor.5d.global.shared::cta.tile.bulk_group [%0, {%2, %3, %4, %5, %6}], [%1];" ::"l"(
          reinterpret_cast<uint64_t>(m)),
      "r"(smem_u32(src)), "r"(c0), "r"(c1), "r"(c2), "r"(c3), "r"(c4)
      : "memory");
}
__device__ __forceinline__ void tma_store_commit() { asm volatile("cp.async.bulk.commit_group;" ::: "memory"); }
__device__ __forceinline__ void tma_store_wait_read0() {
  asm volatile("cp.async.bulk.wait_group.read 0;" ::: "memory");
}
__device__ __forceinline__ void tma_store_wait_all0() { asm volatile("cp.async.bulk.wait_group 0;" ::: "memory"); }

__device__ __forceinline__ void wgmma_fence() { asm volatile("wgmma.fence.sync.aligned;" ::: "memory"); }
__device__ __forceinline__ void wgmma_commit() { asm volatile("wgmma.commit_group.sync.aligned;" ::: "memory"); }
template <int N>
__device__ __forceinline__ void wgmma_wait() { asm volatile("wgmma.wait_group.sync.aligned %0;" ::"n"(N) : "memory"); }

__device__ __forceinline__ uint32_t desc_lo(uint32_t saddr) { return ((saddr >> 4) & 0x3FFFu) | (1u << 16); }
static constexpr uint32_t kDescHiSw128 = (1024u >> 4) | (1u << 30);
__device__ __forceinline__ uint64_t desc_of(uint32_t lo) { return (static_cast<uint64_t>(kDescHiSw128) << 32) | lo; }


__device__ __forceinline__ void named_bar_sync(uint32_t id, uint32_t nthreads) {
  asm volatile("bar.sync %0, %1;" ::"r"(id), "r"(nthreads) : "memory");
}

}
```

deep-image-prior_b200/csrc/wgmma.cuh:

```cuda
#pragma once
#include <stdint.h>

namespace dip {

__device__ __forceinline__ void wgmma_tf32_n32(float (&d)[16], uint64_t a, uint64_t b) {
  asm volatile("{\n\t.reg .pred p;\n\tsetp.ne.b32 p, %18, 0;\n\t"
               "wgmma.mma_async.sync.aligned.m64n32k8.f32.tf32.tf32 {%0, %1, %2, %3, %4, %5, %6, %7, %8, %9, %10, %11, %12, %13, %14, %15}, %16, %17, p, 1, 1;\n\t}\n"
               : "+f"(d[0]), "+f"(d[1]), "+f"(d[2]), "+f"(d[3]), "+f"(d[4]), "+f"(d[5]), "+f"(d[6]), "+f"(d[7]), "+f"(d[8]), "+f"(d[9]), "+f"(d[10]), "+f"(d[11]), "+f"(d[12]), "+f"(d[13]), "+f"(d[14]), "+f"(d[15])
               : "l"(a), "l"(b), "r"(1) : "memory");
}
__device__ __forceinline__ void wgmma_tf32_n64(float (&d)[32], uint64_t a, uint64_t b) {
  asm volatile("{\n\t.reg .pred p;\n\tsetp.ne.b32 p, %34, 0;\n\t"
               "wgmma.mma_async.sync.aligned.m64n64k8.f32.tf32.tf32 {%0, %1, %2, %3, %4, %5, %6, %7, %8, %9, %10, %11, %12, %13, %14, %15, %16, %17, %18, %19, %20, %21, %22, %23, %24, %25, %26, %27, %28, %29, %30, %31}, %32, %33, p, 1, 1;\n\t}\n"
               : "+f"(d[0]), "+f"(d[1]), "+f"(d[2]), "+f"(d[3]), "+f"(d[4]), "+f"(d[5]), "+f"(d[6]), "+f"(d[7]), "+f"(d[8]), "+f"(d[9]), "+f"(d[10]), "+f"(d[11]), "+f"(d[12]), "+f"(d[13]), "+f"(d[14]), "+f"(d[15]), "+f"(d[16]), "+f"(d[17]), "+f"(d[18]), "+f"(d[19]), "+f"(d[20]), "+f"(d[21]), "+f"(d[22]), "+f"(d[23]), "+f"(d[24]), "+f"(d[25]), "+f"(d[26]), "+f"(d[27]), "+f"(d[28]), "+f"(d[29]), "+f"(d[30]), "+f"(d[31])
               : "l"(a), "l"(b), "r"(1) : "memory");
}
__device__ __forceinline__ void wgmma_tf32_n96(float (&d)[48], uint64_t a, uint64_t b) {
  asm volatile("{\n\t.reg .pred p;\n\tsetp.ne.b32 p, %50, 0;\n\t"
               "wgmma.mma_async.sync.aligned.m64n96k8.f32.tf32.tf32 {%0, %1, %2, %3, %4, %5, %6, %7, %8, %9, %10, %11, %12, %13, %14, %15, %16, %17, %18, %19, %20, %21, %22, %23, %24, %25, %26, %27, %28, %29, %30, %31, %32, %33, %34, %35, %36, %37, %38, %39, %40, %41, %42, %43, %44, %45, %46, %47}, %48, %49, p, 1, 1;\n\t}\n"
               : "+f"(d[0]), "+f"(d[1]), "+f"(d[2]), "+f"(d[3]), "+f"(d[4]), "+f"(d[5]), "+f"(d[6]), "+f"(d[7]), "+f"(d[8]), "+f"(d[9]), "+f"(d[10]), "+f"(d[11]), "+f"(d[12]), "+f"(d[13]), "+f"(d[14]), "+f"(d[15]), "+f"(d[16]), "+f"(d[17]), "+f"(d[18]), "+f"(d[19]), "+f"(d[20]), "+f"(d[21]), "+f"(d[22]), "+f"(d[23]), "+f"(d[24]), "+f"(d[25]), "+f"(d[26]), "+f"(d[27]), "+f"(d[28]), "+f"(d[29]), "+f"(d[30]), "+f"(d[31]), "+f"(d[32]), "+f"(d[33]), "+f"(d[34]), "+f"(d[35]), "+f"(d[36]), "+f"(d[37]), "+f"(d[38]), "+f"(d[39]), "+f"(d[40]), "+f"(d[41]), "+f"(d[42]), "+f"(d[43]), "+f"(d[44]), "+f"(d[45]), "+f"(d[46]), "+f"(d[47])
               : "l"(a), "l"(b), "r"(1) : "memory");
}
__device__ __forceinline__ void wgmma_tf32_n128(float (&d)[64], uint64_t a, uint64_t b) {
  asm volatile("{\n\t.reg .pred p;\n\tsetp.ne.b32 p, %66, 0;\n\t"
               "wgmma.mma_async.sync.aligned.m64n128k8.f32.tf32.tf32 {%0, %1, %2, %3, %4, %5, %6, %7, %8, %9, %10, %11, %12, %13, %14, %15, %16, %17, %18, %19, %20, %21, %22, %23, %24, %25, %26, %27, %28, %29, %30, %31, %32, %33, %34, %35, %36, %37, %38, %39, %40, %41, %42, %43, %44, %45, %46, %47, %48, %49, %50, %51, %52, %53, %54, %55, %56, %57, %58, %59, %60, %61, %62, %63}, %64, %65, p, 1, 1;\n\t}\n"
               : "+f"(d[0]), "+f"(d[1]), "+f"(d[2]), "+f"(d[3]), "+f"(d[4]), "+f"(d[5]), "+f"(d[6]), "+f"(d[7]), "+f"(d[8]), "+f"(d[9]), "+f"(d[10]), "+f"(d[11]), "+f"(d[12]), "+f"(d[13]), "+f"(d[14]), "+f"(d[15]), "+f"(d[16]), "+f"(d[17]), "+f"(d[18]), "+f"(d[19]), "+f"(d[20]), "+f"(d[21]), "+f"(d[22]), "+f"(d[23]), "+f"(d[24]), "+f"(d[25]), "+f"(d[26]), "+f"(d[27]), "+f"(d[28]), "+f"(d[29]), "+f"(d[30]), "+f"(d[31]), "+f"(d[32]), "+f"(d[33]), "+f"(d[34]), "+f"(d[35]), "+f"(d[36]), "+f"(d[37]), "+f"(d[38]), "+f"(d[39]), "+f"(d[40]), "+f"(d[41]), "+f"(d[42]), "+f"(d[43]), "+f"(d[44]), "+f"(d[45]), "+f"(d[46]), "+f"(d[47]), "+f"(d[48]), "+f"(d[49]), "+f"(d[50]), "+f"(d[51]), "+f"(d[52]), "+f"(d[53]), "+f"(d[54]), "+f"(d[55]), "+f"(d[56]), "+f"(d[57]), "+f"(d[58]), "+f"(d[59]), "+f"(d[60]), "+f"(d[61]), "+f"(d[62]), "+f"(d[63])
               : "l"(a), "l"(b), "r"(1) : "memory");
}
__device__ __forceinline__ void wgmma_tf32_n160(float (&d)[80], uint64_t a, uint64_t b) {
  asm volatile("{\n\t.reg .pred p;\n\tsetp.ne.b32 p, %82, 0;\n\t"
               "wgmma.mma_async.sync.aligned.m64n160k8.f32.tf32.tf32 {%0, %1, %2, %3, %4, %5, %6, %7, %8, %9, %10, %11, %12, %13, %14, %15, %16, %17, %18, %19, %20, %21, %22, %23, %24, %25, %26, %27, %28, %29, %30, %31, %32, %33, %34, %35, %36, %37, %38, %39, %40, %41, %42, %43, %44, %45, %46, %47, %48, %49, %50, %51, %52, %53, %54, %55, %56, %57, %58, %59, %60, %61, %62, %63, %64, %65, %66, %67, %68, %69, %70, %71, %72, %73, %74, %75, %76, %77, %78, %79}, %80, %81, p, 1, 1;\n\t}\n"
               : "+f"(d[0]), "+f"(d[1]), "+f"(d[2]), "+f"(d[3]), "+f"(d[4]), "+f"(d[5]), "+f"(d[6]), "+f"(d[7]), "+f"(d[8]), "+f"(d[9]), "+f"(d[10]), "+f"(d[11]), "+f"(d[12]), "+f"(d[13]), "+f"(d[14]), "+f"(d[15]), "+f"(d[16]), "+f"(d[17]), "+f"(d[18]), "+f"(d[19]), "+f"(d[20]), "+f"(d[21]), "+f"(d[22]), "+f"(d[23]), "+f"(d[24]), "+f"(d[25]), "+f"(d[26]), "+f"(d[27]), "+f"(d[28]), "+f"(d[29]), "+f"(d[30]), "+f"(d[31]), "+f"(d[32]), "+f"(d[33]), "+f"(d[34]), "+f"(d[35]), "+f"(d[36]), "+f"(d[37]), "+f"(d[38]), "+f"(d[39]), "+f"(d[40]), "+f"(d[41]), "+f"(d[42]), "+f"(d[43]), "+f"(d[44]), "+f"(d[45]), "+f"(d[46]), "+f"(d[47]), "+f"(d[48]), "+f"(d[49]), "+f"(d[50]), "+f"(d[51]), "+f"(d[52]), "+f"(d[53]), "+f"(d[54]), "+f"(d[55]), "+f"(d[56]), "+f"(d[57]), "+f"(d[58]), "+f"(d[59]), "+f"(d[60]), "+f"(d[61]), "+f"(d[62]), "+f"(d[63]), "+f"(d[64]), "+f"(d[65]), "+f"(d[66]), "+f"(d[67]), "+f"(d[68]), "+f"(d[69]), "+f"(d[70]), "+f"(d[71]), "+f"(d[72]), "+f"(d[73]), "+f"(d[74]), "+f"(d[75]), "+f"(d[76]), "+f"(d[77]), "+f"(d[78]), "+f"(d[79])
               : "l"(a), "l"(b), "r"(1) : "memory");
}
__device__ __forceinline__ void wgmma_bf16_n32(float (&d)[16], uint64_t a, uint64_t b) {
  asm volatile("{\n\t.reg .pred p;\n\tsetp.ne.b32 p, %18, 0;\n\t"
               "wgmma.mma_async.sync.aligned.m64n32k16.f32.bf16.bf16 {%0, %1, %2, %3, %4, %5, %6, %7, %8, %9, %10, %11, %12, %13, %14, %15}, %16, %17, p, 1, 1, 0, 0;\n\t}\n"
               : "+f"(d[0]), "+f"(d[1]), "+f"(d[2]), "+f"(d[3]), "+f"(d[4]), "+f"(d[5]), "+f"(d[6]), "+f"(d[7]), "+f"(d[8]), "+f"(d[9]), "+f"(d[10]), "+f"(d[11]), "+f"(d[12]), "+f"(d[13]), "+f"(d[14]), "+f"(d[15])
               : "l"(a), "l"(b), "r"(1) : "memory");
}
__device__ __forceinline__ void wgmma_bf16_n64(float (&d)[32], uint64_t a, uint64_t b) {
  asm volatile("{\n\t.reg .pred p;\n\tsetp.ne.b32 p, %34, 0;\n\t"
               "wgmma.mma_async.sync.aligned.m64n64k16.f32.bf16.bf16 {%0, %1, %2, %3, %4, %5, %6, %7, %8, %9, %10, %11, %12, %13, %14, %15, %16, %17, %18, %19, %20, %21, %22, %23, %24, %25, %26, %27, %28, %29, %30, %31}, %32, %33, p, 1, 1, 0, 0;\n\t}\n"
               : "+f"(d[0]), "+f"(d[1]), "+f"(d[2]), "+f"(d[3]), "+f"(d[4]), "+f"(d[5]), "+f"(d[6]), "+f"(d[7]), "+f"(d[8]), "+f"(d[9]), "+f"(d[10]), "+f"(d[11]), "+f"(d[12]), "+f"(d[13]), "+f"(d[14]), "+f"(d[15]), "+f"(d[16]), "+f"(d[17]), "+f"(d[18]), "+f"(d[19]), "+f"(d[20]), "+f"(d[21]), "+f"(d[22]), "+f"(d[23]), "+f"(d[24]), "+f"(d[25]), "+f"(d[26]), "+f"(d[27]), "+f"(d[28]), "+f"(d[29]), "+f"(d[30]), "+f"(d[31])
               : "l"(a), "l"(b), "r"(1) : "memory");
}
__device__ __forceinline__ void wgmma_bf16_n96(float (&d)[48], uint64_t a, uint64_t b) {
  asm volatile("{\n\t.reg .pred p;\n\tsetp.ne.b32 p, %50, 0;\n\t"
               "wgmma.mma_async.sync.aligned.m64n96k16.f32.bf16.bf16 {%0, %1, %2, %3, %4, %5, %6, %7, %8, %9, %10, %11, %12, %13, %14, %15, %16, %17, %18, %19, %20, %21, %22, %23, %24, %25, %26, %27, %28, %29, %30, %31, %32, %33, %34, %35, %36, %37, %38, %39, %40, %41, %42, %43, %44, %45, %46, %47}, %48, %49, p, 1, 1, 0, 0;\n\t}\n"
               : "+f"(d[0]), "+f"(d[1]), "+f"(d[2]), "+f"(d[3]), "+f"(d[4]), "+f"(d[5]), "+f"(d[6]), "+f"(d[7]), "+f"(d[8]), "+f"(d[9]), "+f"(d[10]), "+f"(d[11]), "+f"(d[12]), "+f"(d[13]), "+f"(d[14]), "+f"(d[15]), "+f"(d[16]), "+f"(d[17]), "+f"(d[18]), "+f"(d[19]), "+f"(d[20]), "+f"(d[21]), "+f"(d[22]), "+f"(d[23]), "+f"(d[24]), "+f"(d[25]), "+f"(d[26]), "+f"(d[27]), "+f"(d[28]), "+f"(d[29]), "+f"(d[30]), "+f"(d[31]), "+f"(d[32]), "+f"(d[33]), "+f"(d[34]), "+f"(d[35]), "+f"(d[36]), "+f"(d[37]), "+f"(d[38]), "+f"(d[39]), "+f"(d[40]), "+f"(d[41]), "+f"(d[42]), "+f"(d[43]), "+f"(d[44]), "+f"(d[45]), "+f"(d[46]), "+f"(d[47])
               : "l"(a), "l"(b), "r"(1) : "memory");
}
__device__ __forceinline__ void wgmma_bf16_n128(float (&d)[64], uint64_t a, uint64_t b) {
  asm volatile("{\n\t.reg .pred p;\n\tsetp.ne.b32 p, %66, 0;\n\t"
               "wgmma.mma_async.sync.aligned.m64n128k16.f32.bf16.bf16 {%0, %1, %2, %3, %4, %5, %6, %7, %8, %9, %10, %11, %12, %13, %14, %15, %16, %17, %18, %19, %20, %21, %22, %23, %24, %25, %26, %27, %28, %29, %30, %31, %32, %33, %34, %35, %36, %37, %38, %39, %40, %41, %42, %43, %44, %45, %46, %47, %48, %49, %50, %51, %52, %53, %54, %55, %56, %57, %58, %59, %60, %61, %62, %63}, %64, %65, p, 1, 1, 0, 0;\n\t}\n"
               : "+f"(d[0]), "+f"(d[1]), "+f"(d[2]), "+f"(d[3]), "+f"(d[4]), "+f"(d[5]), "+f"(d[6]), "+f"(d[7]), "+f"(d[8]), "+f"(d[9]), "+f"(d[10]), "+f"(d[11]), "+f"(d[12]), "+f"(d[13]), "+f"(d[14]), "+f"(d[15]), "+f"(d[16]), "+f"(d[17]), "+f"(d[18]), "+f"(d[19]), "+f"(d[20]), "+f"(d[21]), "+f"(d[22]), "+f"(d[23]), "+f"(d[24]), "+f"(d[25]), "+f"(d[26]), "+f"(d[27]), "+f"(d[28]), "+f"(d[29]), "+f"(d[30]), "+f"(d[31]), "+f"(d[32]), "+f"(d[33]), "+f"(d[34]), "+f"(d[35]), "+f"(d[36]), "+f"(d[37]), "+f"(d[38]), "+f"(d[39]), "+f"(d[40]), "+f"(d[41]), "+f"(d[42]), "+f"(d[43]), "+f"(d[44]), "+f"(d[45]), "+f"(d[46]), "+f"(d[47]), "+f"(d[48]), "+f"(d[49]), "+f"(d[50]), "+f"(d[51]), "+f"(d[52]), "+f"(d[53]), "+f"(d[54]), "+f"(d[55]), "+f"(d[56]), "+f"(d[57]), "+f"(d[58]), "+f"(d[59]), "+f"(d[60]), "+f"(d[61]), "+f"(d[62]), "+f"(d[63])
               : "l"(a), "l"(b), "r"(1) : "memory");
}
__device__ __forceinline__ void wgmma_bf16_n136(float (&d)[68], uint64_t a, uint64_t b) {
  asm volatile("{\n\t.reg .pred p;\n\tsetp.ne.b32 p, %70, 0;\n\t"
               "wgmma.mma_async.sync.aligned.m64n136k16.f32.bf16.bf16 {%0, %1, %2, %3, %4, %5, %6, %7, %8, %9, %10, %11, %12, %13, %14, %15, %16, %17, %18, %19, %20, %21, %22, %23, %24, %25, %26, %27, %28, %29, %30, %31, %32, %33, %34, %35, %36, %37, %38, %39, %40, %41, %42, %43, %44, %45, %46, %47, %48, %49, %50, %51, %52, %53, %54, %55, %56, %57, %58, %59, %60, %61, %62, %63, %64, %65, %66, %67}, %68, %69, p, 1, 1, 0, 0;\n\t}\n"
               : "+f"(d[0]), "+f"(d[1]), "+f"(d[2]), "+f"(d[3]), "+f"(d[4]), "+f"(d[5]), "+f"(d[6]), "+f"(d[7]), "+f"(d[8]), "+f"(d[9]), "+f"(d[10]), "+f"(d[11]), "+f"(d[12]), "+f"(d[13]), "+f"(d[14]), "+f"(d[15]), "+f"(d[16]), "+f"(d[17]), "+f"(d[18]), "+f"(d[19]), "+f"(d[20]), "+f"(d[21]), "+f"(d[22]), "+f"(d[23]), "+f"(d[24]), "+f"(d[25]), "+f"(d[26]), "+f"(d[27]), "+f"(d[28]), "+f"(d[29]), "+f"(d[30]), "+f"(d[31]), "+f"(d[32]), "+f"(d[33]), "+f"(d[34]), "+f"(d[35]), "+f"(d[36]), "+f"(d[37]), "+f"(d[38]), "+f"(d[39]), "+f"(d[40]), "+f"(d[41]), "+f"(d[42]), "+f"(d[43]), "+f"(d[44]), "+f"(d[45]), "+f"(d[46]), "+f"(d[47]), "+f"(d[48]), "+f"(d[49]), "+f"(d[50]), "+f"(d[51]), "+f"(d[52]), "+f"(d[53]), "+f"(d[54]), "+f"(d[55]), "+f"(d[56]), "+f"(d[57]), "+f"(d[58]), "+f"(d[59]), "+f"(d[60]), "+f"(d[61]), "+f"(d[62]), "+f"(d[63]), "+f"(d[64]), "+f"(d[65]), "+f"(d[66]), "+f"(d[67])
               : "l"(a), "l"(b), "r"(1) : "memory");
}
__device__ __forceinline__ void wgmma_bf16_n160(float (&d)[80], uint64_t a, uint64_t b) {
  asm volatile("{\n\t.reg .pred p;\n\tsetp.ne.b32 p, %82, 0;\n\t"
               "wgmma.mma_async.sync.aligned.m64n160k16.f32.bf16.bf16 {%0, %1, %2, %3, %4, %5, %6, %7, %8, %9, %10, %11, %12, %13, %14, %15, %16, %17, %18, %19, %20, %21, %22, %23, %24, %25, %26, %27, %28, %29, %30, %31, %32, %33, %34, %35, %36, %37, %38, %39, %40, %41, %42, %43, %44, %45, %46, %47, %48, %49, %50, %51, %52, %53, %54, %55, %56, %57, %58, %59, %60, %61, %62, %63, %64, %65, %66, %67, %68, %69, %70, %71, %72, %73, %74, %75, %76, %77, %78, %79}, %80, %81, p, 1, 1, 0, 0;\n\t}\n"
               : "+f"(d[0]), "+f"(d[1]), "+f"(d[2]), "+f"(d[3]), "+f"(d[4]), "+f"(d[5]), "+f"(d[6]), "+f"(d[7]), "+f"(d[8]), "+f"(d[9]), "+f"(d[10]), "+f"(d[11]), "+f"(d[12]), "+f"(d[13]), "+f"(d[14]), "+f"(d[15]), "+f"(d[16]), "+f"(d[17]), "+f"(d[18]), "+f"(d[19]), "+f"(d[20]), "+f"(d[21]), "+f"(d[22]), "+f"(d[23]), "+f"(d[24]), "+f"(d[25]), "+f"(d[26]), "+f"(d[27]), "+f"(d[28]), "+f"(d[29]), "+f"(d[30]), "+f"(d[31]), "+f"(d[32]), "+f"(d[33]), "+f"(d[34]), "+f"(d[35]), "+f"(d[36]), "+f"(d[37]), "+f"(d[38]), "+f"(d[39]), "+f"(d[40]), "+f"(d[41]), "+f"(d[42]), "+f"(d[43]), "+f"(d[44]), "+f"(d[45]), "+f"(d[46]), "+f"(d[47]), "+f"(d[48]), "+f"(d[49]), "+f"(d[50]), "+f"(d[51]), "+f"(d[52]), "+f"(d[53]), "+f"(d[54]), "+f"(d[55]), "+f"(d[56]), "+f"(d[57]), "+f"(d[58]), "+f"(d[59]), "+f"(d[60]), "+f"(d[61]), "+f"(d[62]), "+f"(d[63]), "+f"(d[64]), "+f"(d[65]), "+f"(d[66]), "+f"(d[67]), "+f"(d[68]), "+f"(d[69]), "+f"(d[70]), "+f"(d[71]), "+f"(d[72]), "+f"(d[73]), "+f"(d[74]), "+f"(d[75]), "+f"(d[76]), "+f"(d[77]), "+f"(d[78]), "+f"(d[79])
               : "l"(a), "l"(b), "r"(1) : "memory");
}

__device__ __forceinline__ void wgmma_tf32_rs_n32(float (&d)[16], const uint32_t (&a)[4], uint64_t b) {
  asm volatile("{\n\t.reg .pred p;\n\tsetp.ne.b32 p, %21, 0;\n\t"
               "wgmma.mma_async.sync.aligned.m64n32k8.f32.tf32.tf32 {%0, %1, %2, %3, %4, %5, %6, %7, %8, %9, %10, %11, %12, %13, %14, %15}, {%16, %17, %18, %19}, %20, p, 1, 1;\n\t}\n"
               : "+f"(d[0]), "+f"(d[1]), "+f"(d[2]), "+f"(d[3]), "+f"(d[4]), "+f"(d[5]), "+f"(d[6]), "+f"(d[7]), "+f"(d[8]), "+f"(d[9]), "+f"(d[10]), "+f"(d[11]), "+f"(d[12]), "+f"(d[13]), "+f"(d[14]), "+f"(d[15])
               : "r"(a[0]), "r"(a[1]), "r"(a[2]), "r"(a[3]), "l"(b), "r"(1) : "memory");
}
__device__ __forceinline__ void wgmma_tf32_rs_n64(float (&d)[32], const uint32_t (&a)[4], uint64_t b) {
  asm volatile("{\n\t.reg .pred p;\n\tsetp.ne.b32 p, %37, 0;\n\t"
               "wgmma.mma_async.sync.aligned.m64n64k8.f32.tf32.tf32 {%0, %1, %2, %3, %4, %5, %6, %7, %8, %9, %10, %11, %12, %13, %14, %15, %16, %17, %18, %19, %20, %21, %22, %23, %24, %25, %26, %27, %28, %29, %30, %31}, {%32, %33, %34, %35}, %36, p, 1, 1;\n\t}\n"
               : "+f"(d[0]), "+f"(d[1]), "+f"(d[2]), "+f"(d[3]), "+f"(d[4]), "+f"(d[5]), "+f"(d[6]), "+f"(d[7]), "+f"(d[8]), "+f"(d[9]), "+f"(d[10]), "+f"(d[11]), "+f"(d[12]), "+f"(d[13]), "+f"(d[14]), "+f"(d[15]), "+f"(d[16]), "+f"(d[17]), "+f"(d[18]), "+f"(d[19]), "+f"(d[20]), "+f"(d[21]), "+f"(d[22]), "+f"(d[23]), "+f"(d[24]), "+f"(d[25]), "+f"(d[26]), "+f"(d[27]), "+f"(d[28]), "+f"(d[29]), "+f"(d[30]), "+f"(d[31])
               : "r"(a[0]), "r"(a[1]), "r"(a[2]), "r"(a[3]), "l"(b), "r"(1) : "memory");
}
__device__ __forceinline__ void wgmma_tf32_rs_n96(float (&d)[48], const uint32_t (&a)[4], uint64_t b) {
  asm volatile("{\n\t.reg .pred p;\n\tsetp.ne.b32 p, %53, 0;\n\t"
               "wgmma.mma_async.sync.aligned.m64n96k8.f32.tf32.tf32 {%0, %1, %2, %3, %4, %5, %6, %7, %8, %9, %10, %11, %12, %13, %14, %15, %16, %17, %18, %19, %20, %21, %22, %23, %24, %25, %26, %27, %28, %29, %30, %31, %32, %33, %34, %35, %36, %37, %38, %39, %40, %41, %42, %43, %44, %45, %46, %47}, {%48, %49, %50, %51}, %52, p, 1, 1;\n\t}\n"
               : "+f"(d[0]), "+f"(d[1]), "+f"(d[2]), "+f"(d[3]), "+f"(d[4]), "+f"(d[5]), "+f"(d[6]), "+f"(d[7]), "+f"(d[8]), "+f"(d[9]), "+f"(d[10]), "+f"(d[11]), "+f"(d[12]), "+f"(d[13]), "+f"(d[14]), "+f"(d[15]), "+f"(d[16]), "+f"(d[17]), "+f"(d[18]), "+f"(d[19]), "+f"(d[20]), "+f"(d[21]), "+f"(d[22]), "+f"(d[23]), "+f"(d[24]), "+f"(d[25]), "+f"(d[26]), "+f"(d[27]), "+f"(d[28]), "+f"(d[29]), "+f"(d[30]), "+f"(d[31]), "+f"(d[32]), "+f"(d[33]), "+f"(d[34]), "+f"(d[35]), "+f"(d[36]), "+f"(d[37]), "+f"(d[38]), "+f"(d[39]), "+f"(d[40]), "+f"(d[41]), "+f"(d[42]), "+f"(d[43]), "+f"(d[44]), "+f"(d[45]), "+f"(d[46]), "+f"(d[47])
               : "r"(a[0]), "r"(a[1]), "r"(a[2]), "r"(a[3]), "l"(b), "r"(1) : "memory");
}
__device__ __forceinline__ void wgmma_tf32_rs_n128(float (&d)[64], const uint32_t (&a)[4], uint64_t b) {
  asm volatile("{\n\t.reg .pred p;\n\tsetp.ne.b32 p, %69, 0;\n\t"
               "wgmma.mma_async.sync.aligned.m64n128k8.f32.tf32.tf32 {%0, %1, %2, %3, %4, %5, %6, %7, %8, %9, %10, %11, %12, %13, %14, %15, %16, %17, %18, %19, %20, %21, %22, %23, %24, %25, %26, %27, %28, %29, %30, %31, %32, %33, %34, %35, %36, %37, %38, %39, %40, %41, %42, %43, %44, %45, %46, %47, %48, %49, %50, %51, %52, %53, %54, %55, %56, %57, %58, %59, %60, %61, %62, %63}, {%64, %65, %66, %67}, %68, p, 1, 1;\n\t}\n"
               : "+f"(d[0]), "+f"(d[1]), "+f"(d[2]), "+f"(d[3]), "+f"(d[4]), "+f"(d[5]), "+f"(d[6]), "+f"(d[7]), "+f"(d[8]), "+f"(d[9]), "+f"(d[10]), "+f"(d[11]), "+f"(d[12]), "+f"(d[13]), "+f"(d[14]), "+f"(d[15]), "+f"(d[16]), "+f"(d[17]), "+f"(d[18]), "+f"(d[19]), "+f"(d[20]), "+f"(d[21]), "+f"(d[22]), "+f"(d[23]), "+f"(d[24]), "+f"(d[25]), "+f"(d[26]), "+f"(d[27]), "+f"(d[28]), "+f"(d[29]), "+f"(d[30]), "+f"(d[31]), "+f"(d[32]), "+f"(d[33]), "+f"(d[34]), "+f"(d[35]), "+f"(d[36]), "+f"(d[37]), "+f"(d[38]), "+f"(d[39]), "+f"(d[40]), "+f"(d[41]), "+f"(d[42]), "+f"(d[43]), "+f"(d[44]), "+f"(d[45]), "+f"(d[46]), "+f"(d[47]), "+f"(d[48]), "+f"(d[49]), "+f"(d[50]), "+f"(d[51]), "+f"(d[52]), "+f"(d[53]), "+f"(d[54]), "+f"(d[55]), "+f"(d[56]), "+f"(d[57]), "+f"(d[58]), "+f"(d[59]), "+f"(d[60]), "+f"(d[61]), "+f"(d[62]), "+f"(d[63])
               : "r"(a[0]), "r"(a[1]), "r"(a[2]), "r"(a[3]), "l"(b), "r"(1) : "memory");
}
__device__ __forceinline__ void wgmma_tf32_rs_n136(float (&d)[68], const uint32_t (&a)[4], uint64_t b) {
  asm volatile("{\n\t.reg .pred p;\n\tsetp.ne.b32 p, %73, 0;\n\t"
               "wgmma.mma_async.sync.aligned.m64n136k8.f32.tf32.tf32 {%0, %1, %2, %3, %4, %5, %6, %7, %8, %9, %10, %11, %12, %13, %14, %15, %16, %17, %18, %19, %20, %21, %22, %23, %24, %25, %26, %27, %28, %29, %30, %31, %32, %33, %34, %35, %36, %37, %38, %39, %40, %41, %42, %43, %44, %45, %46, %47, %48, %49, %50, %51, %52, %53, %54, %55, %56, %57, %58, %59, %60, %61, %62, %63, %64, %65, %66, %67}, {%68, %69, %70, %71}, %72, p, 1, 1;\n\t}\n"
               : "+f"(d[0]), "+f"(d[1]), "+f"(d[2]), "+f"(d[3]), "+f"(d[4]), "+f"(d[5]), "+f"(d[6]), "+f"(d[7]), "+f"(d[8]), "+f"(d[9]), "+f"(d[10]), "+f"(d[11]), "+f"(d[12]), "+f"(d[13]), "+f"(d[14]), "+f"(d[15]), "+f"(d[16]), "+f"(d[17]), "+f"(d[18]), "+f"(d[19]), "+f"(d[20]), "+f"(d[21]), "+f"(d[22]), "+f"(d[23]), "+f"(d[24]), "+f"(d[25]), "+f"(d[26]), "+f"(d[27]), "+f"(d[28]), "+f"(d[29]), "+f"(d[30]), "+f"(d[31]), "+f"(d[32]), "+f"(d[33]), "+f"(d[34]), "+f"(d[35]), "+f"(d[36]), "+f"(d[37]), "+f"(d[38]), "+f"(d[39]), "+f"(d[40]), "+f"(d[41]), "+f"(d[42]), "+f"(d[43]), "+f"(d[44]), "+f"(d[45]), "+f"(d[46]), "+f"(d[47]), "+f"(d[48]), "+f"(d[49]), "+f"(d[50]), "+f"(d[51]), "+f"(d[52]), "+f"(d[53]), "+f"(d[54]), "+f"(d[55]), "+f"(d[56]), "+f"(d[57]), "+f"(d[58]), "+f"(d[59]), "+f"(d[60]), "+f"(d[61]), "+f"(d[62]), "+f"(d[63]), "+f"(d[64]), "+f"(d[65]), "+f"(d[66]), "+f"(d[67])
               : "r"(a[0]), "r"(a[1]), "r"(a[2]), "r"(a[3]), "l"(b), "r"(1) : "memory");
}
__device__ __forceinline__ void wgmma_tf32_rs_n160(float (&d)[80], const uint32_t (&a)[4], uint64_t b) {
  asm volatile("{\n\t.reg .pred p;\n\tsetp.ne.b32 p, %85, 0;\n\t"
               "wgmma.mma_async.sync.aligned.m64n160k8.f32.tf32.tf32 {%0, %1, %2, %3, %4, %5, %6, %7, %8, %9, %10, %11, %12, %13, %14, %15, %16, %17, %18, %19, %20, %21, %22, %23, %24, %25, %26, %27, %28, %29, %30, %31, %32, %33, %34, %35, %36, %37, %38, %39, %40, %41, %42, %43, %44, %45, %46, %47, %48, %49, %50, %51, %52, %53, %54, %55, %56, %57, %58, %59, %60, %61, %62, %63, %64, %65, %66, %67, %68, %69, %70, %71, %72, %73, %74, %75, %76, %77, %78, %79}, {%80, %81, %82, %83}, %84, p, 1, 1;\n\t}\n"
               : "+f"(d[0]), "+f"(d[1]), "+f"(d[2]), "+f"(d[3]), "+f"(d[4]), "+f"(d[5]), "+f"(d[6]), "+f"(d[7]), "+f"(d[8]), "+f"(d[9]), "+f"(d[10]), "+f"(d[11]), "+f"(d[12]), "+f"(d[13]), "+f"(d[14]), "+f"(d[15]), "+f"(d[16]), "+f"(d[17]), "+f"(d[18]), "+f"(d[19]), "+f"(d[20]), "+f"(d[21]), "+f"(d[22]), "+f"(d[23]), "+f"(d[24]), "+f"(d[25]), "+f"(d[26]), "+f"(d[27]), "+f"(d[28]), "+f"(d[29]), "+f"(d[30]), "+f"(d[31]), "+f"(d[32]), "+f"(d[33]), "+f"(d[34]), "+f"(d[35]), "+f"(d[36]), "+f"(d[37]), "+f"(d[38]), "+f"(d[39]), "+f"(d[40]), "+f"(d[41]), "+f"(d[42]), "+f"(d[43]), "+f"(d[44]), "+f"(d[45]), "+f"(d[46]), "+f"(d[47]), "+f"(d[48]), "+f"(d[49]), "+f"(d[50]), "+f"(d[51]), "+f"(d[52]), "+f"(d[53]), "+f"(d[54]), "+f"(d[55]), "+f"(d[56]), "+f"(d[57]), "+f"(d[58]), "+f"(d[59]), "+f"(d[60]), "+f"(d[61]), "+f"(d[62]), "+f"(d[63]), "+f"(d[64]), "+f"(d[65]), "+f"(d[66]), "+f"(d[67]), "+f"(d[68]), "+f"(d[69]), "+f"(d[70]), "+f"(d[71]), "+f"(d[72]), "+f"(d[73]), "+f"(d[74]), "+f"(d[75]), "+f"(d[76]), "+f"(d[77]), "+f"(d[78]), "+f"(d[79])
               : "r"(a[0]), "r"(a[1]), "r"(a[2]), "r"(a[3]), "l"(b), "r"(1) : "memory");
}

template <int N, bool BF16>
__device__ __forceinline__ void wgmma_ss(float (&d)[N / 2], uint64_t a, uint64_t b) {
  static_assert(N == 32 || N == 64 || N == 96 || N == 128 || (N == 136 && BF16) || N == 160, "wgmma N");
  if constexpr (BF16) {
    if constexpr (N == 32) wgmma_bf16_n32(d, a, b);
    else if constexpr (N == 64) wgmma_bf16_n64(d, a, b);
    else if constexpr (N == 96) wgmma_bf16_n96(d, a, b);
    else if constexpr (N == 128) wgmma_bf16_n128(d, a, b);
    else if constexpr (N == 136) wgmma_bf16_n136(d, a, b);
    else wgmma_bf16_n160(d, a, b);
  } else {
    if constexpr (N == 32) wgmma_tf32_n32(d, a, b);
    else if constexpr (N == 64) wgmma_tf32_n64(d, a, b);
    else if constexpr (N == 96) wgmma_tf32_n96(d, a, b);
    else if constexpr (N == 128) wgmma_tf32_n128(d, a, b);
    else wgmma_tf32_n160(d, a, b);
  }
}

template <int N>
__device__ __forceinline__ void wgmma_rs(float (&d)[N / 2], const uint32_t (&a)[4], uint64_t b) {
  static_assert(N == 32 || N == 64 || N == 96 || N == 128 || N == 136 || N == 160, "wgmma N");
  if constexpr (N == 32) wgmma_tf32_rs_n32(d, a, b);
  else if constexpr (N == 64) wgmma_tf32_rs_n64(d, a, b);
  else if constexpr (N == 96) wgmma_tf32_rs_n96(d, a, b);
  else if constexpr (N == 128) wgmma_tf32_rs_n128(d, a, b);
  else if constexpr (N == 136) wgmma_tf32_rs_n136(d, a, b);
  else wgmma_tf32_rs_n160(d, a, b);
}

}
```

Measured before the change: 190.8.

## Add halo-patch 3x3 conv kernel reusing one input tile across all taps

Adds a tensor-core conv path for 3x3 stride-1 layers. A (bw+2)x(bh+2) input halo patch per channel block is loaded once with a non-swizzled 4D TMA and kept resident in shared memory. All nine taps then index into it with shifted no-swizzle wgmma descriptors, while only the weights stream through the stage pipeline. This is meant to cut the repeated per-tap activation loads of the implicit-GEMM kernel. The cost is extra shared memory, possible bank conflicts from the unswizzled A layout, and new mbarrier bookkeeping. The change also adds an N=144 wgmma variant and factors the epilogue and stats flush into shared helpers.

```diff
diff --git a/deep-image-prior_b200/csrc/conv_tc.cu b/deep-image-prior_b200/csrc/conv_tc.cu
--- a/deep-image-prior_b200/csrc/conv_tc.cu
+++ b/deep-image-prior_b200/csrc/conv_tc.cu
@@ -20,17 +20,21 @@
 __host__ __device__ constexpr int round32(int n) { return (n + 31) & ~31; }
 __host__ __device__ constexpr int round1024(int n) { return (n + 1023) & ~1023; }
 
+template <int NT>
+__device__ __forceinline__ void tc_conv_epilogue(const TcConvParams& p, const TcConvParams* pm, SmemCtl* ctl, uint8_t* staging,
+                                                 float (&acc)[2][NT / 2], int x0, int y0, int opx, int opy, int n_off,
+                                                 double& stat_s1, double& stat_s2, bool col_halves = false);
+__device__ __forceinline__ void tc_conv_stats_flush(const TcConvParams& p, int n_off, double stat_s1, double stat_s2);
+
 template <bool BF16, int NT>
 __device__ __forceinline__ void tc_conv_consumer(const TcConvParams& p, const TcConvParams* pm, SmemCtl* ctl,
                                                  uint8_t* stage_base, int stage_bytes, uint8_t* staging, int n_iters,
                                                  int tile0, int tile_stride, int num_tiles, int tiles_pp, int n_off) {
-  const int et = threadIdx.x - 128;
-  const int w = et >> 5, lane = et & 31;
+  const int lane = threadIdx.x & 31;
   float acc[2][NT / 2];
   int stage = 0;
   uint32_t phase = 0;
   double stat_s1 = 0.0, stat_s2 = 0.0;
-  const int bw_shift = 31 - __clz(p.bw);
   const uint32_t base_lo = desc_lo(smem_u32(stage_base));
   const uint32_t stage_step = static_cast<uint32_t>(stage_bytes) >> 4;
   constexpr uint32_t kBOff = static_cast<uint32_t>(kABytes) >> 4;
@@ -72,7 +76,19 @@
     }
     wgmma_wait<0>();
     if (prev >= 0 && lane == 0) mbar_arrive(&ctl->empty[prev]);
-
+    tc_conv_epilogue<NT>(p, pm, ctl, staging, acc, x0, y0, opx, opy, n_off, stat_s1, stat_s2);
+  }
+  tc_conv_stats_flush(p, n_off, stat_s1, stat_s2);
+}
+
+template <int NT>
+__device__ __forceinline__ void tc_conv_epilogue(const TcConvParams& p, const TcConvParams* pm, SmemCtl* ctl, uint8_t* staging,
+                                                 float (&acc)[2][NT / 2], int x0, int y0, int opx, int opy, int n_off,
+                                                 double& stat_s1, double& stat_s2, bool col_halves) {
+  const int et = threadIdx.x - 128;
+  const int w = et >> 5, lane = et & 31;
+  const int bw_shift = 31 - __clz(p.bw);
+  {
     if (et == 0) tma_store_wait_read0();
     named_bar_sync(1, 128);
 #pragma unroll
@@ -85,7 +101,8 @@
           const int q = (col & 31) >> 2, e = col & 3;
 #pragma unroll
           for (int rr = 0; rr < 2; ++rr) {
-            const int row = 64 * h + 16 * w + (lane >> 2) + 8 * rr;
+            const int r64 = 16 * w + (lane >> 2) + 8 * rr;
+            const int row = col_halves ? ((r64 >> 3) << 4) + 8 * h + (r64 & 7) : 64 * h + r64;
             float2 o;
             o.x = acc[h][4 * j + 2 * rr] + ctl->bias[col];
             o.y = acc[h][4 * j + 2 * rr + 1] + ctl->bias[col + 1];
@@ -129,6 +146,10 @@
       stat_s2 += static_cast<double>(b0 + b1);
     }
   }
+}
+
+__device__ __forceinline__ void tc_conv_stats_flush(const TcConvParams& p, int n_off, double stat_s1, double stat_s2) {
+  const int et = threadIdx.x - 128;
   if (p.stats != nullptr && et < p.n_mma && n_off + et < p.stats_ld) {
     const int rep = (blockIdx.x % kAccR) * kAccLine;
     atomicAdd(&p.stats[(n_off + et) * kAccStride + rep], stat_s1);
@@ -238,6 +259,179 @@
 __global__ void __launch_bounds__(kNumThreads, 1) tc_conv_kernel_bf16(const __grid_constant__ TcConvParams p) {
   extern __shared__ __align__(1024) uint8_t smem_raw[];
   tc_conv_body<false, true>(p, &p, smem_raw);
+}
+
+__host__ __device__ constexpr int patch_nt(int n_mma) { return n_mma == 144 ? 144 : round32(n_mma); }
+struct PatchCtl {
+  uint64_t pfull[kPatchMaxKb];
+  uint64_t pempty[kPatchMaxKb];
+};
+
+struct PatchWork {
+  int tile0, tile_stride, n_iters, n_off, n_total;
+};
+__device__ __forceinline__ PatchWork patch_work(const TcConvParams& p) {
+  const int n_split = p.n_split < 1 ? 1 : p.n_split;
+  PatchWork w;
+  const int num_tiles = p.tiles_x * p.tiles_y;
+  w.tile_stride = static_cast<int>(gridDim.x) / n_split;
+  w.tile0 = blockIdx.x / n_split;
+  w.n_iters = (num_tiles - w.tile0 + w.tile_stride - 1) / w.tile_stride;
+  w.n_off = static_cast<int>(blockIdx.x % n_split) * p.n_mma;
+  w.n_total = p.n_mma * n_split;
+  return w;
+}
+static constexpr int kPatchTaps = 9;
+
+template <bool BF16, int NT>
+__device__ __forceinline__ void tc_conv_patch_consumer(const TcConvParams& p, const TcConvParams* pm, SmemCtl* ctl, PatchCtl* pc,
+                                                       uint8_t* patch_base, uint8_t* b_base, int b_stage_bytes,
+                                                       uint8_t* staging, const PatchWork& wk) {
+  const int lane = threadIdx.x & 31;
+  float acc[2][NT / 2];
+  int stage = 0;
+  uint32_t phase = 0, pphase = 0;
+  double stat_s1 = 0.0, stat_s2 = 0.0;
+  const uint32_t patch16 = smem_u32(patch_base) >> 4;
+  const uint32_t b_lo0 = desc_lo(smem_u32(b_base));
+  const uint32_t b_step = static_cast<uint32_t>(b_stage_bytes) >> 4;
+  constexpr uint32_t kPlane16 = kPatchPlane >> 4, kSlot16 = kPatchBytes >> 4;
+  const uint32_t row16 = p.bw + 2;
+  const uint32_t half16 = p.bw == 8 ? 8 * row16 : 8;
+  for (int it = 0; it < wk.n_iters; ++it) {
+    const int tile = wk.tile0 + it * wk.tile_stride;
+    const int x0 = (tile % p.tiles_x) * p.bw, y0 = (tile / p.tiles_x) * p.bh;
+#pragma unroll
+    for (int i = 0; i < NT / 2; ++i) { acc[0][i] = 0.f; acc[1][i] = 0.f; }
+    int prev = -1;
+    int prev_patch = -1;
+#pragma unroll 1
+    for (int tap = 0; tap < kPatchTaps; ++tap) {
+      const int r = tap / 3, s = tap - 3 * (tap / 3);
+#pragma unroll 1
+      for (int kb = 0; kb < p.kblocks; ++kb) {
+        if (tap == 0) mbar_wait(&pc->pfull[kb], pphase);
+        mbar_wait(&ctl->full[stage], phase);
+        const uint32_t b_lo = b_lo0 + stage * b_step;
+        const uint32_t a16 = patch16 + kb * kSlot16 + r * row16 + s;
+        wgmma_fence();
+#pragma unroll
+        for (int k = 0; k < 4; ++k) {
+          wgmma_ss<NT, BF16>(acc[0], desc_noswz(a16 + 2 * k * kPlane16, kPlane16, row16), desc_of(b_lo + 2 * k));
+          wgmma_ss<NT, BF16>(acc[1], desc_noswz(a16 + half16 + 2 * k * kPlane16, kPlane16, row16), desc_of(b_lo + 2 * k));
+        }
+        wgmma_commit();
+        if (prev >= 0) {
+          wgmma_wait<1>();
+          if (lane == 0) {
+            mbar_arrive(&ctl->empty[prev]);
+            if (prev_patch >= 0) mbar_arrive(&pc->pempty[prev_patch]);
+          }
+        }
+        prev = stage;
+        prev_patch = tap == kPatchTaps - 1 ? kb : -1;
+        if (++stage == p.stages) { stage = 0; phase ^= 1; }
+      }
+    }
+    pphase ^= 1;
+    wgmma_wait<0>();
+    if (prev >= 0 && lane == 0) {
+      mbar_arrive(&ctl->empty[prev]);
+      if (prev_patch >= 0) mbar_arrive(&pc->pempty[prev_patch]);
+    }
+    tc_conv_epilogue<NT>(p, pm, ctl, staging, acc, x0, y0, 0, 0, wk.n_off, stat_s1, stat_s2, p.bw == 16);
+  }
+  tc_conv_stats_flush(p, wk.n_off, stat_s1, stat_s2);
+}
+
+template <bool BF16>
+__device__ __forceinline__ void tc_conv_patch_body(const TcConvParams& p, uint8_t* smem_raw) {
+  constexpr int KE = BF16 ? 64 : 32;
+  constexpr int KG = BF16 ? 8 : 4;
+  uint8_t* smem = reinterpret_cast<uint8_t*>((reinterpret_cast<uintptr_t>(smem_raw) + 1023) & ~uintptr_t(1023));
+  const int nt = patch_nt(p.n_mma);
+  const int b_bytes = p.n_mma * 128;
+  const int b_stage_bytes = round1024(nt * 128);
+  uint8_t* b_base = smem;
+  uint8_t* staging = b_base + p.stages * b_stage_bytes;
+  uint8_t* patch_base = staging + p.n_chunks * kChunkBytes;
+  SmemCtl* ctl = reinterpret_cast<SmemCtl*>(patch_base + p.kblocks * kPatchBytes);
+  PatchCtl* pc = reinterpret_cast<PatchCtl*>(ctl + 1);
+
+  const int warp = threadIdx.x >> 5;
+  const int lane = threadIdx.x & 31;
+  const PatchWork wk = patch_work(p);
+
+  pdl_trigger();
+  if (warp == 0 && lane == 0) {
+    tma_prefetch_desc(&p.tmA);
+    tma_prefetch_desc(&p.tmB);
+    tma_prefetch_desc(&p.tmD);
+  }
+  if (warp == 1 && lane == 0) {
+    for (int i = 0; i < p.stages; ++i) {
+      mbar_init(&ctl->full[i], 1);
+      mbar_init(&ctl->empty[i], 4);
+    }
+    for (int i = 0; i < p.kblocks; ++i) {
+      mbar_init(&pc->pfull[i], 1);
+      mbar_init(&pc->pempty[i], 4);
+    }
+    fence_mbar_init();
+  }
+  pdl_wait();
+  if (warp == 3) {
+    for (int i = lane; i < 160; i += 32)
+      ctl->bias[i] = (p.bias != nullptr && i < p.n_mma && (p.n_valid == 0 || wk.n_off + i < p.n_valid)) ? p.bias[wk.n_off + i] : 0.f;
+  }
+  __syncthreads();
+
+  if (warp == 0) {
+    int stage = 0;
+    uint32_t phase = 0, pphase = 0;
+    for (int it = 0; it < wk.n_iters; ++it) {
+      const int tile = wk.tile0 + it * wk.tile_stride;
+      const int x0 = (tile % p.tiles_x) * p.bw, y0 = (tile / p.tiles_x) * p.bh;
+      for (int tap = 0; tap < kPatchTaps; ++tap) {
+        for (int kb = 0; kb < p.kblocks; ++kb) {
+          if (tap == 0) {
+            mbar_wait(&pc->pempty[kb], pphase ^ 1);
+            if (elect_one()) {
+              mbar_expect_tx(&pc->pfull[kb], kPatchBytes);
+              tma_load_4d(patch_base + kb * kPatchBytes, &p.tmA, &pc->pfull[kb], 0, x0 + p.offx, y0 + p.offy, kb * (KE / KG));
+            }
+            __syncwarp();
+          }
+          mbar_wait(&ctl->empty[stage], phase ^ 1);
+          if (elect_one()) {
+            mbar_expect_tx(&ctl->full[stage], b_bytes);
+            tma_load_2d(b_base + stage * b_stage_bytes, &p.tmB, &ctl->full[stage], kb * KE, tap * wk.n_total + wk.n_off);
+          }
+          __syncwarp();
+          if (++stage == p.stages) { stage = 0; phase ^= 1; }
+        }
+      }
+      pphase ^= 1;
+    }
+  } else if (warp >= 4) {
+    switch (nt) {
+      case 32: tc_conv_patch_consumer<BF16, 32>(p, &p, ctl, pc, patch_base, b_base, b_stage_bytes, staging, wk); break;
+      case 64: tc_conv_patch_consumer<BF16, 64>(p, &p, ctl, pc, patch_base, b_base, b_stage_bytes, staging, wk); break;
+      case 96: tc_conv_patch_consumer<BF16, 96>(p, &p, ctl, pc, patch_base, b_base, b_stage_bytes, staging, wk); break;
+      case 128: tc_conv_patch_consumer<BF16, 128>(p, &p, ctl, pc, patch_base, b_base, b_stage_bytes, staging, wk); break;
+      case 144: tc_conv_patch_consumer<BF16, 144>(p, &p, ctl, pc, patch_base, b_base, b_stage_bytes, staging, wk); break;
+      default: tc_conv_patch_consumer<BF16, 160>(p, &p, ctl, pc, patch_base, b_base, b_stage_bytes, staging, wk); break;
+    }
+  }
+  __syncthreads();
+}
+__global__ void __launch_bounds__(kNumThreads, 1) tc_conv_patch_kernel(const __grid_constant__ TcConvParams p) {
+  extern __shared__ __align__(1024) uint8_t smem_raw[];
+  tc_conv_patch_body<false>(p, smem_raw);
+}
+__global__ void __launch_bounds__(kNumThreads, 1) tc_conv_patch_kernel_bf16(const __grid_constant__ TcConvParams p) {
+  extern __shared__ __align__(1024) uint8_t smem_raw[];
+  tc_conv_patch_body<true>(p, smem_raw);
 }
 
 struct SmemCtlW {
@@ -575,7 +769,10 @@
 static constexpr size_t kMaxSmem = 232448;
 
 size_t tc_conv_smem_bytes(const TcConvParams& p) {
-  const size_t b_bytes = round1024(round32(p.n_mma) * 128);
+  const size_t b_bytes = round1024((p.patch ? patch_nt(p.n_mma) : round32(p.n_mma)) * 128);
+  if (p.patch)
+    return 1024 + p.stages * b_bytes + static_cast<size_t>(p.n_chunks) * kChunkBytes +
+           static_cast<size_t>(p.kblocks) * kPatchBytes + sizeof(SmemCtl) + sizeof(PatchCtl);
   return 1024 + p.stages * (kABytes + b_bytes) + static_cast<size_t>(p.n_chunks) * kChunkBytes + sizeof(SmemCtl);
 }
 size_t tc_wgrad_smem_bytes(const TcWgradParams& p) {
@@ -589,6 +786,10 @@
   if (e != cudaSuccess) return e;
   e = cudaFuncSetAttribute(tc_conv_kernel_bf16, cudaFuncAttributeMaxDynamicSharedMemorySize, (int)kMaxSmem);
   if (e != cudaSuccess) return e;
+  e = cudaFuncSetAttribute(tc_conv_patch_kernel, cudaFuncAttributeMaxDynamicSharedMemorySize, (int)kMaxSmem);
+  if (e != cudaSuccess) return e;
+  e = cudaFuncSetAttribute(tc_conv_patch_kernel_bf16, cudaFuncAttributeMaxDynamicSharedMemorySize, (int)kMaxSmem);
+  if (e != cudaSuccess) return e;
   e = cudaFuncSetAttribute(tc_wgrad_kernel_bf16, cudaFuncAttributeMaxDynamicSharedMemorySize, (int)kMaxSmem);
   if (e != cudaSuccess) return e;
   return cudaFuncSetAttribute(tc_wgrad_kernel, cudaFuncAttributeMaxDynamicSharedMemorySize, (int)kMaxSmem);
@@ -597,7 +798,8 @@
 static bool conv_params_ok(const TcConvParams& p) {
   return p.n_mma >= 1 && p.n_mma <= 160 && p.n_chunks == (p.n_mma + 31) / 32 && p.stages >= 1 && p.stages <= 8 &&
          p.kblocks >= 1 && p.nphase >= 0 && p.nphase <= 4 &&
-         (p.bw & (p.bw - 1)) == 0 && p.bw * p.bh == kTileM;
+         (p.bw & (p.bw - 1)) == 0 && p.bw * p.bh == kTileM &&
+         (!p.patch || (((p.bw == 8 && p.bh == 16) || (p.bw == 16 && p.bh == 8)) && p.kblocks <= kPatchMaxKb && p.kh == 3 && p.kw == 3 && p.stride == 1 && p.nphase == 0));
 }
 
 cudaError_t tc_conv_launch(const TcConvParams& p, int num_sms, cudaStream_t s) {
@@ -610,6 +812,8 @@
   }
   const size_t smem = tc_conv_smem_bytes(p);
   if (smem > kMaxSmem) return cudaErrorInvalidValue;
+  if (p.patch)
+    return launch_k(p.bf16 ? tc_conv_patch_kernel_bf16 : tc_conv_patch_kernel, dim3(grid), dim3(kNumThreads), smem, s, 1, p);
   return launch_k(p.bf16 ? tc_conv_kernel_bf16 : tc_conv_kernel, dim3(grid), dim3(kNumThreads), smem, s, 1, p);
 }
 int tc_conv_grid(const TcConvParams& p, int num_sms) {
diff --git a/deep-image-prior_b200/csrc/conv_tc.cuh b/deep-image-prior_b200/csrc/conv_tc.cuh
--- a/deep-image-prior_b200/csrc/conv_tc.cuh
+++ b/deep-image-prior_b200/csrc/conv_tc.cuh
@@ -28,7 +28,11 @@
   const float* bias;
   double* stats;
   int stats_ld;
+  int patch;
 };
+static constexpr int kPatchPlane = 180 * 16;
+static constexpr int kPatchMaxKb = 8;
+static constexpr int kPatchBytes = 8 * kPatchPlane;
 
 static constexpr int kWgradKp = 32;
 struct TcWgradParams {
diff --git a/deep-image-prior_b200/csrc/engine.cu b/deep-image-prior_b200/csrc/engine.cu
--- a/deep-image-prior_b200/csrc/engine.cu
+++ b/deep-image-prior_b200/csrc/engine.cu
@@ -66,10 +66,10 @@
 static bool is_tc(int prec) { return prec == DIP_PRECISION_TF32 || prec == DIP_PRECISION_BF16; }
 
 static int encode_map(CUtensorMap* m, const void* base, int rank, const cuuint64_t* dims, const cuuint64_t* strides_b,
-                      const cuuint32_t* box, bool bf16 = false) {
+                      const cuuint32_t* box, bool bf16 = false, bool swizzle = true) {
   cuuint32_t estr[5] = {1, 1, 1, 1, 1};
   CUresult r = g_encode(m, bf16 ? CU_TENSOR_MAP_DATA_TYPE_BFLOAT16 : CU_TENSOR_MAP_DATA_TYPE_FLOAT32, rank, const_cast<void*>(base), dims, strides_b, box, estr,
-                        CU_TENSOR_MAP_INTERLEAVE_NONE, CU_TENSOR_MAP_SWIZZLE_128B,
+                        CU_TENSOR_MAP_INTERLEAVE_NONE, swizzle ? CU_TENSOR_MAP_SWIZZLE_128B : CU_TENSOR_MAP_SWIZZLE_NONE,
                         CU_TENSOR_MAP_L2_PROMOTION_L2_128B,
                         CU_TENSOR_MAP_FLOAT_OOB_FILL_NONE);
   if (r != CUDA_SUCCESS) {
@@ -101,6 +101,14 @@
   cuuint64_t str[2] = {ld * e, (cuuint64_t)cols * ld * e};
   cuuint32_t box[3] = {bf16 ? 64u : 32u, (cuuint32_t)bw, (cuuint32_t)bh};
   return encode_map(m, base, 3, dims, str, box, bf16);
+}
+static int map_patch(CUtensorMap* m, const void* base, int rows, int cols, int ld, int c, int bw, int bh, bool bf16) {
+  const cuuint64_t e = bf16 ? 2 : sizeof(float);
+  const cuuint64_t g = 16 / e;
+  cuuint64_t dims[4] = {g, (cuuint64_t)cols, (cuuint64_t)rows, (cuuint64_t)c / g};
+  cuuint64_t str[3] = {ld * e, (cuuint64_t)cols * ld * e, 16};
+  cuuint32_t box[4] = {(cuuint32_t)g, (cuuint32_t)bw + 2, (cuuint32_t)bh + 2, 8};
+  return encode_map(m, base, 4, dims, str, box, bf16, false);
 }
 static int map_w2(CUtensorMap* m, const void* base, int rows_total, int kcols, int box_rows, bool bf16 = false) {
   const cuuint64_t e = bf16 ? 2 : sizeof(float);
@@ -159,7 +167,7 @@
   return sp;
 }
 static void fit_stages(TcConvParams& p, size_t budget = 232448) {
-  p.stages = 6;
+  p.stages = p.patch ? 8 : 6;
   while (tc_conv_smem_bytes(p) > budget && p.stages > 2) p.stages--;
 }
 struct ConvOp {
@@ -191,6 +199,7 @@
   const float* wg_dy = nullptr; int wg_h = 0, wg_w = 0;
   int p_w = -1, p_b = -1;
   TcConvParams fp{}, dg{};
+  TcConvParams fp_run{}, dg_run{};
   TcWgradParams wg{};
   int simt_ksplits = 1;
 
@@ -216,6 +225,17 @@
     return is_tc(prec) ? wacc_elems() : (size_t)simt_ksplits * k * k * 128 * c_pad;
   }
 
+  int patch_form(const TcConvParams& g, TcConvParams& q, const void* act, int rows, int cols, int ld, int kc) {
+    q = g;
+    if ((g.bw != 8 && g.bw != 16) || kc % (bf16 ? 8 : 4) != 0 || g.kblocks > kPatchMaxKb) return 0;
+    TcConvParams t = g;
+    t.patch = 1;
+    fit_stages(t);
+    if (tc_conv_smem_bytes(t) > 232448) return 0;
+    DIP_CHECK(map_patch(&t.tmA, act, rows, cols, ld, kc, g.bw, g.bh, bf16));
+    q = t;
+    return 0;
+  }
   int build_tc(float* partial) {
     int bw, bh;
     pick_tile(out_w, out_h, &bw, &bh);
@@ -236,6 +256,9 @@
     fp.bias = nullptr; fp.stats = stats; fp.stats_ld = N;
     fit_stages(fp);
     }
+    fp_run = fp;
+    if (do_fprop && k == 3 && stride == 1)
+      DIP_CHECK(bf16 ? patch_form(fp, fp_run, in16, in_rows, in_cols, in_ld16, C) : patch_form(fp, fp_run, in, in_rows, in_cols, in_ld, C));
     if (has_dgrad && dg_s2) {
       const int gh = dg_out_h / 2, gw = dg_out_w / 2;
       pick_tile(gw, gh, &bw, &bh);
@@ -278,6 +301,9 @@
       dg.bias = nullptr; dg.stats = nullptr; dg.stats_ld = 0;
       fit_stages(dg);
     }
+    dg_run = dg;
+    if (has_dgrad && !dg_s2 && k == 3)
+      DIP_CHECK(bf16 ? patch_form(dg, dg_run, dg_in16, dg_in_h, dg_in_w, N, N) : patch_form(dg, dg_run, dg_in, dg_in_h, dg_in_w, N, N));
     wg = TcWgradParams{};
     if (!do_wgrad) return 0;
     wg.bf16 = bf16 ? 1 : 0;
@@ -303,7 +329,7 @@
 
   int run_fprop(int prec, const float* bias, cudaStream_t s) {
     if (is_tc(prec)) {
-      TcConvParams p = fp;
+      TcConvParams p = fp_run;
       p.bias = bias;
       TimeScope ts(timer, 0, alg_flops(), s);
       DIP_CUDA(tc_conv_launch(p, g_num_sms, s));
@@ -322,7 +348,7 @@
   int run_dgrad(int prec, cudaStream_t s) {
     if (is_tc(prec)) {
       TimeScope ts(timer, 1, alg_flops(), s);
-      DIP_CUDA(tc_conv_launch(dg, g_num_sms, s));
+      DIP_CUDA(tc_conv_launch(dg_run, g_num_sms, s));
     } else {
       SimtConvArgs a{};
       a.A = dg_in; a.a_h = dg_in_h; a.a_w = dg_in_w; a.a_ld = N; a.a_c = N;
diff --git a/deep-image-prior_b200/csrc/ptx.cuh b/deep-image-prior_b200/csrc/ptx.cuh
--- a/deep-image-prior_b200/csrc/ptx.cuh
+++ b/deep-image-prior_b200/csrc/ptx.cuh
@@ -80,6 +80,14 @@
       "l"(reinterpret_cast<uint64_t>(m)), "r"(smem_u32(bar)), "r"(c0), "r"(c1), "r"(c2)
       : "memory");
 }
+__device__ __forceinline__ void tma_load_4d(void* dst, const CUtensorMap* m, uint64_t* bar, int c0, int c1,
+                                            int c2, int c3) {
+  asm volatile(
+      "cp.async.bulk.tensor.4d.shared::cluster.global.tile.mbarrier::complete_tx::bytes "
+      "[%0], [%1, {%3, %4, %5, %6}], [%2];" ::"r"(smem_u32(dst)),
+      "l"(reinterpret_cast<uint64_t>(m)), "r"(smem_u32(bar)), "r"(c0), "r"(c1), "r"(c2), "r"(c3)
+      : "memory");
+}
 __device__ __forceinline__ void tma_load_5d(void* dst, const CUtensorMap* m, uint64_t* bar, int c0, int c1,
                                             int c2, int c3, int c4) {
   asm volatile(
@@ -117,6 +125,11 @@
 static constexpr uint32_t kDescHiSw128 = (1024u >> 4) | (1u << 30);
 __device__ __forceinline__ uint64_t desc_of(uint32_t lo) { return (static_cast<uint64_t>(kDescHiSw128) << 32) | lo; }
 
+__host__ __device__ constexpr uint64_t desc_noswz(uint32_t start16, uint32_t lbo16, uint32_t sbo16) {
+  return static_cast<uint64_t>(start16 & 0x3FFFu) | (static_cast<uint64_t>(lbo16 & 0x3FFFu) << 16) |
+         (static_cast<uint64_t>(sbo16 & 0x3FFFu) << 32);
+}
+
 
 __device__ __forceinline__ void named_bar_sync(uint32_t id, uint32_t nthreads) {
   asm volatile("bar.sync %0, %1;" ::"r"(id), "r"(nthreads) : "memory");
diff --git a/deep-image-prior_b200/csrc/wgmma.cuh b/deep-image-prior_b200/csrc/wgmma.cuh
--- a/deep-image-prior_b200/csrc/wgmma.cuh
+++ b/deep-image-prior_b200/csrc/wgmma.cuh
@@ -25,6 +25,12 @@
   asm volatile("{\n\t.reg .pred p;\n\tsetp.ne.b32 p, %66, 0;\n\t"
                "wgmma.mma_async.sync.aligned.m64n128k8.f32.tf32.tf32 {%0, %1, %2, %3, %4, %5, %6, %7, %8, %9, %10, %11, %12, %13, %14, %15, %16, %17, %18, %19, %20, %21, %22, %23, %24, %25, %26, %27, %28, %29, %30, %31, %32, %33, %34, %35, %36, %37, %38, %39, %40, %41, %42, %43, %44, %45, %46, %47, %48, %49, %50, %51, %52, %53, %54, %55, %56, %57, %58, %59, %60, %61, %62, %63}, %64, %65, p, 1, 1;\n\t}\n"
                : "+f"(d[0]), "+f"(d[1]), "+f"(d[2]), "+f"(d[3]), "+f"(d[4]), "+f"(d[5]), "+f"(d[6]), "+f"(d[7]), "+f"(d[8]), "+f"(d[9]), "+f"(d[10]), "+f"(d[11]), "+f"(d[12]), "+f"(d[13]), "+f"(d[14]), "+f"(d[15]), "+f"(d[16]), "+f"(d[17]), "+f"(d[18]), "+f"(d[19]), "+f"(d[20]), "+f"(d[21]), "+f"(d[22]), "+f"(d[23]), "+f"(d[24]), "+f"(d[25]), "+f"(d[26]), "+f"(d[27]), "+f"(d[28]), "+f"(d[29]), "+f"(d[30]), "+f"(d[31]), "+f"(d[32]), "+f"(d[33]), "+f"(d[34]), "+f"(d[35]), "+f"(d[36]), "+f"(d[37]), "+f"(d[38]), "+f"(d[39]), "+f"(d[40]), "+f"(d[41]), "+f"(d[42]), "+f"(d[43]), "+f"(d[44]), "+f"(d[45]), "+f"(d[46]), "+f"(d[47]), "+f"(d[48]), "+f"(d[49]), "+f"(d[50]), "+f"(d[51]), "+f"(d[52]), "+f"(d[53]), "+f"(d[54]), "+f"(d[55]), "+f"(d[56]), "+f"(d[57]), "+f"(d[58]), "+f"(d[59]), "+f"(d[60]), "+f"(d[61]), "+f"(d[62]), "+f"(d[63])
+               : "l"(a), "l"(b), "r"(1) : "memory");
+}
+__device__ __forceinline__ void wgmma_tf32_n144(float (&d)[72], uint64_t a, uint64_t b) {
+  asm volatile("{\n\t.reg .pred p;\n\tsetp.ne.b32 p, %74, 0;\n\t"
+               "wgmma.mma_async.sync.aligned.m64n144k8.f32.tf32.tf32 {%0, %1, %2, %3, %4, %5, %6, %7, %8, %9, %10, %11, %12, %13, %14, %15, %16, %17, %18, %19, %20, %21, %22, %23, %24, %25, %26, %27, %28, %29, %30, %31, %32, %33, %34, %35, %36, %37, %38, %39, %40, %41, %42, %43, %44, %45, %46, %47, %48, %49, %50, %51, %52, %53, %54, %55, %56, %57, %58, %59, %60, %61, %62, %63, %64, %65, %66, %67, %68, %69, %70, %71}, %72, %73, p, 1, 1;\n\t}\n"
+               : "+f"(d[0]), "+f"(d[1]), "+f"(d[2]), "+f"(d[3]), "+f"(d[4]), "+f"(d[5]), "+f"(d[6]), "+f"(d[7]), "+f"(d[8]), "+f"(d[9]), "+f"(d[10]), "+f"(d[11]), "+f"(d[12]), "+f"(d[13]), "+f"(d[14]), "+f"(d[15]), "+f"(d[16]), "+f"(d[17]), "+f"(d[18]), "+f"(d[19]), "+f"(d[20]), "+f"(d[21]), "+f"(d[22]), "+f"(d[23]), "+f"(d[24]), "+f"(d[25]), "+f"(d[26]), "+f"(d[27]), "+f"(d[28]), "+f"(d[29]), "+f"(d[30]), "+f"(d[31]), "+f"(d[32]), "+f"(d[33]), "+f"(d[34]), "+f"(d[35]), "+f"(d[36]), "+f"(d[37]), "+f"(d[38]), "+f"(d[39]), "+f"(d[40]), "+f"(d[41]), "+f"(d[42]), "+f"(d[43]), "+f"(d[44]), "+f"(d[45]), "+f"(d[46]), "+f"(d[47]), "+f"(d[48]), "+f"(d[49]), "+f"(d[50]), "+f"(d[51]), "+f"(d[52]), "+f"(d[53]), "+f"(d[54]), "+f"(d[55]), "+f"(d[56]), "+f"(d[57]), "+f"(d[58]), "+f"(d[59]), "+f"(d[60]), "+f"(d[61]), "+f"(d[62]), "+f"(d[63]), "+f"(d[64]), "+f"(d[65]), "+f"(d[66]), "+f"(d[67]), "+f"(d[68]), "+f"(d[69]), "+f"(d[70]), "+f"(d[71])
                : "l"(a), "l"(b), "r"(1) : "memory");
 }
 __device__ __forceinline__ void wgmma_tf32_n160(float (&d)[80], uint64_t a, uint64_t b) {
@@ -61,6 +67,12 @@
   asm volatile("{\n\t.reg .pred p;\n\tsetp.ne.b32 p, %70, 0;\n\t"
                "wgmma.mma_async.sync.aligned.m64n136k16.f32.bf16.bf16 {%0, %1, %2, %3, %4, %5, %6, %7, %8, %9, %10, %11, %12, %13, %14, %15, %16, %17, %18, %19, %20, %21, %22, %23, %24, %25, %26, %27, %28, %29, %30, %31, %32, %33, %34, %35, %36, %37, %38, %39, %40, %41, %42, %43, %44, %45, %46, %47, %48, %49, %50, %51, %52, %53, %54, %55, %56, %57, %58, %59, %60, %61, %62, %63, %64, %65, %66, %67}, %68, %69, p, 1, 1, 0, 0;\n\t}\n"
                : "+f"(d[0]), "+f"(d[1]), "+f"(d[2]), "+f"(d[3]), "+f"(d[4]), "+f"(d[5]), "+f"(d[6]), "+f"(d[7]), "+f"(d[8]), "+f"(d[9]), "+f"(d[10]), "+f"(d[11]), "+f"(d[12]), "+f"(d[13]), "+f"(d[14]), "+f"(d[15]), "+f"(d[16]), "+f"(d[17]), "+f"(d[18]), "+f"(d[19]), "+f"(d[20]), "+f"(d[21]), "+f"(d[22]), "+f"(d[23]), "+f"(d[24]), "+f"(d[25]), "+f"(d[26]), "+f"(d[27]), "+f"(d[28]), "+f"(d[29]), "+f"(d[30]), "+f"(d[31]), "+f"(d[32]), "+f"(d[33]), "+f"(d[34]), "+f"(d[35]), "+f"(d[36]), "+f"(d[37]), "+f"(d[38]), "+f"(d[39]), "+f"(d[40]), "+f"(d[41]), "+f"(d[42]), "+f"(d[43]), "+f"(d[44]), "+f"(d[45]), "+f"(d[46]), "+f"(d[47]), "+f"(d[48]), "+f"(d[49]), "+f"(d[50]), "+f"(d[51]), "+f"(d[52]), "+f"(d[53]), "+f"(d[54]), "+f"(d[55]), "+f"(d[56]), "+f"(d[57]), "+f"(d[58]), "+f"(d[59]), "+f"(d[60]), "+f"(d[61]), "+f"(d[62]), "+f"(d[63]), "+f"(d[64]), "+f"(d[65]), "+f"(d[66]), "+f"(d[67])
+               : "l"(a), "l"(b), "r"(1) : "memory");
+}
+__device__ __forceinline__ void wgmma_bf16_n144(float (&d)[72], uint64_t a, uint64_t b) {
+  asm volatile("{\n\t.reg .pred p;\n\tsetp.ne.b32 p, %74, 0;\n\t"
+               "wgmma.mma_async.sync.aligned.m64n144k16.f32.bf16.bf16 {%0, %1, %2, %3, %4, %5, %6, %7, %8, %9, %10, %11, %12, %13, %14, %15, %16, %17, %18, %19, %20, %21, %22, %23, %24, %25, %26, %27, %28, %29, %30, %31, %32, %33, %34, %35, %36, %37, %38, %39, %40, %41, %42, %43, %44, %45, %46, %47, %48, %49, %50, %51, %52, %53, %54, %55, %56, %57, %58, %59, %60, %61, %62, %63, %64, %65, %66, %67, %68, %69, %70, %71}, %72, %73, p, 1, 1, 0, 0;\n\t}\n"
+               : "+f"(d[0]), "+f"(d[1]), "+f"(d[2]), "+f"(d[3]), "+f"(d[4]), "+f"(d[5]), "+f"(d[6]), "+f"(d[7]), "+f"(d[8]), "+f"(d[9]), "+f"(d[10]), "+f"(d[11]), "+f"(d[12]), "+f"(d[13]), "+f"(d[14]), "+f"(d[15]), "+f"(d[16]), "+f"(d[17]), "+f"(d[18]), "+f"(d[19]), "+f"(d[20]), "+f"(d[21]), "+f"(d[22]), "+f"(d[23]), "+f"(d[24]), "+f"(d[25]), "+f"(d[26]), "+f"(d[27]), "+f"(d[28]), "+f"(d[29]), "+f"(d[30]), "+f"(d[31]), "+f"(d[32]), "+f"(d[33]), "+f"(d[34]), "+f"(d[35]), "+f"(d[36]), "+f"(d[37]), "+f"(d[38]), "+f"(d[39]), "+f"(d[40]), "+f"(d[41]), "+f"(d[42]), "+f"(d[43]), "+f"(d[44]), "+f"(d[45]), "+f"(d[46]), "+f"(d[47]), "+f"(d[48]), "+f"(d[49]), "+f"(d[50]), "+f"(d[51]), "+f"(d[52]), "+f"(d[53]), "+f"(d[54]), "+f"(d[55]), "+f"(d[56]), "+f"(d[57]), "+f"(d[58]), "+f"(d[59]), "+f"(d[60]), "+f"(d[61]), "+f"(d[62]), "+f"(d[63]), "+f"(d[64]), "+f"(d[65]), "+f"(d[66]), "+f"(d[67]), "+f"(d[68]), "+f"(d[69]), "+f"(d[70]), "+f"(d[71])
                : "l"(a), "l"(b), "r"(1) : "memory");
 }
 __device__ __forceinline__ void wgmma_bf16_n160(float (&d)[80], uint64_t a, uint64_t b) {
@@ -109,19 +121,21 @@
 
 template <int N, bool BF16>
 __device__ __forceinline__ void wgmma_ss(float (&d)[N / 2], uint64_t a, uint64_t b) {
-  static_assert(N == 32 || N == 64 || N == 96 || N == 128 || (N == 136 && BF16) || N == 160, "wgmma N");
+  static_assert(N == 32 || N == 64 || N == 96 || N == 128 || (N == 136 && BF16) || N == 144 || N == 160, "wgmma N");
   if constexpr (BF16) {
     if constexpr (N == 32) wgmma_bf16_n32(d, a, b);
     else if constexpr (N == 64) wgmma_bf16_n64(d, a, b);
     else if constexpr (N == 96) wgmma_bf16_n96(d, a, b);
     else if constexpr (N == 128) wgmma_bf16_n128(d, a, b);
     else if constexpr (N == 136) wgmma_bf16_n136(d, a, b);
+    else if constexpr (N == 144) wgmma_bf16_n144(d, a, b);
     else wgmma_bf16_n160(d, a, b);
   } else {
     if constexpr (N == 32) wgmma_tf32_n32(d, a, b);
     else if constexpr (N == 64) wgmma_tf32_n64(d, a, b);
     else if constexpr (N == 96) wgmma_tf32_n96(d, a, b);
     else if constexpr (N == 128) wgmma_tf32_n128(d, a, b);
+    else if constexpr (N == 144) wgmma_tf32_n144(d, a, b);
     else wgmma_tf32_n160(d, a, b);
   }
 }
```

New measurement: 202.8 (median of 6 runs). 1.06x the previous value.
